# jy-yuan/KIVI

Measured on NVIDIA H100. Metric: decode tokens/sec @ Llama-2-7B bs32 seq4k K2V2, higher is better.
Workload: dtype f16 (fp32 accumulate; 2-bit K / 2-bit V codes)

## Files before the change

include/kivi_b200.h:

```cpp
#ifndef KIVI_B200_H
#define KIVI_B200_H

#include <stdint.h>

#ifdef __cplusplus
extern "C" {
#endif

#define KIVI_OK              0
#define KIVI_ERR_BITS       -1
#define KIVI_ERR_SHAPE      -2
#define KIVI_ERR_GQA        -3
#define KIVI_ERR_GROUP      -4
#define KIVI_ERR_ALIGN      -5
#define KIVI_ERR_NULL       -6
#define KIVI_ERR_LAYOUT     -7
#define KIVI_ERR_CAPACITY   -8
#define KIVI_ERR_UNSUPPORTED -9

#define KIVI_LAYOUT_REFERENCE 0
#define KIVI_LAYOUT_KERNEL    1

int         kivi_version(void);
const char* kivi_error_string(int code);
uint64_t    kivi_launch_count(void);

int kivi_pack_lastdim_f16(const void* x, int64_t rows, int64_t T, int group_size, int bits,
                          void* code, void* scale, void* mn, void* stream);

int kivi_bgemv_outer_f16(const void* A, int64_t a_stride,
                         const void* qB, int64_t qb_unit_stride, int64_t qb_row_stride,
                         const void* scales, const void* zeros, int64_t sz_unit_stride, int64_t sz_row_stride,
                         void* C, int B, int nh, int nh_kv, int K, int N,
                         int bits, int group_size, int layout, void* stream);

int kivi_gemv_inner_f16(const void* in, const void* kernel, const void* scales, const void* zeros,
                        void* out, int Bn, int IC, int OC, int bits, int group_size, int64_t sf_w,
                        void* stream);

int kivi_unpack_dequant_lastdim_f16(const void* code, const void* scale, const void* mn,
                                    int64_t rows, int64_t T, int group_size, int bits,
                                    void* out, void* stream);

#define KIVI_CACHE_OVERLAP_PROLOGUE 1
#define KIVI_CACHE_GQA_CHUNK_SHIFT 4
#define KIVI_CACHE_GQA_CHUNK(g)    ((g) << KIVI_CACHE_GQA_CHUNK_SHIFT)

typedef struct kivi_cache {
    int32_t batch, num_heads, num_kv_heads, head_dim;
    int32_t k_bits, v_bits, group_size, residual_length;
    int32_t k_cap_blocks;
    int32_t v_cap_blocks;
    int32_t v_res_cap;
    int32_t flags;
    void* k_store;
    void* v_store;
    void* k_res;
    void* v_res;
    void* state;
} kivi_cache_t;

int kivi_cache_sizes(int batch, int num_kv_heads, int k_bits, int v_bits, int group_size,
                     int residual_length, int max_tokens, int64_t* out);

int kivi_cache_prefill_f16(const kivi_cache_t* cache, const void* k, const void* v, int n, void* stream);

int64_t kivi_decode_workspace_bytes(const kivi_cache_t* cache, int max_kv_len);

int kivi_decode_attention_f16(const kivi_cache_t* cache, const void* q, const void* k_new, const void* v_new,
                              const void* mask, void* out, void* workspace, int64_t workspace_bytes,
                              void* dbg_logits, void* dbg_probs, int64_t dbg_stride, int max_kv_len, void* stream);

int kivi_decode_attention_ragged_f16(const kivi_cache_t* cache, const void* q, const void* k_new, const void* v_new,
                                     const int32_t* kv_start, const void* mask, void* out, void* workspace,
                                     int64_t workspace_bytes, void* dbg_logits, void* dbg_probs, int64_t dbg_stride,
                                     int max_kv_len, void* stream);

int kivi_debug_range_split(int n_units, int n_b, int n_w, int w_cap, int kernel, int* out_lo, int* out_owner);

int kivi_debug_ragged_items(int n_units, int n_b, int n_w, int w_cap, int kernel, const int* unit_start, int kv_len,
                            int* issued, int* consumed, int64_t cap, int64_t* n_out);

int kivi_cache_advance(const kivi_cache_t* cache, void* stream);

#define KIVI_STATE_ERR_CAPACITY 1
#define KIVI_STATE_ERR_LENGTHS  2
int kivi_cache_read_state(const kivi_cache_t* cache, int32_t* host_state8, void* stream);

int kivi_cache_refill_f16(const kivi_cache_t* cache, int seq, const void* k, const void* v, int n,
                          int tk, int r, int tv, int L, int vhead, void* stream);

int kivi_cache_shift_f16(const kivi_cache_t* cache, int shift, int tk, int tv, void* stream);

int kivi_cache_shift_state(const kivi_cache_t* cache, int shift, int32_t* kv_start, void* stream);

int kivi_cache_export_f16(const kivi_cache_t* cache, int tk, int r, int tv, int L, int vhead,
                          void* k_code, void* k_scale, void* k_mn, void* k_full,
                          void* v_code, void* v_scale, void* v_mn, void* v_full, void* stream);

int kivi_cache_import_f16(const kivi_cache_t* cache, int tk, int r, int tv, int L,
                          const void* k_code, const void* k_scale, const void* k_mn, const void* k_full,
                          const void* v_code, const void* v_scale, const void* v_mn, const void* v_full, void* stream);

int kivi_add_rmsnorm_f16(const void* x, void* residual, const void* weight, void* out,
                         int rows, int hidden, float eps, void* stream);
int kivi_rope_split_f16(const void* qkv, const void* cos_table, const void* sin_table, const void* pos,
                        void* q, void* k, void* v, int batch, int num_heads, int num_kv_heads, int table_rows,
                        void* stream);
int kivi_silu_mul_f16(const void* gate_up, void* out, int rows, int intermediate, void* stream);

int kivi_greedy_sample_exchange_f32(const void* logits, int batch, int vocab, void* next_local, void* ids_feedback,
                                    const void* peer_buffers, int rank, int world, const void* step, void* err, void* stream);

#ifdef __cplusplus
}
#endif
#endif
```

kivi_b200/csrc/kivi_attn.cuh:

```cuda
#pragma once
#include <cstdlib>
#include "kivi_decode.cuh"

#ifndef KIVI_UNROLL
#define KIVI_UNROLL 8
#endif
constexpr int kChunkUnroll = KIVI_UNROLL;
#ifndef KIVI_Z_SIMT
#define KIVI_Z_SIMT 0
#endif
#ifndef KIVI_EVICT_FIRST
#define KIVI_EVICT_FIRST 1
#endif
#ifndef KIVI_SHIFT_IMAD
#define KIVI_SHIFT_IMAD 0
#endif
#ifndef KIVI_PRED_FINALIZE
#define KIVI_PRED_FINALIZE 1
#endif
#ifndef KIVI_EARLY_COMMIT
#define KIVI_EARLY_COMMIT 1
#endif
#ifndef KIVI_UNIT_FLAGS
#define KIVI_UNIT_FLAGS 0
#endif
#ifndef KIVI_COMMIT_IN_QK
#define KIVI_COMMIT_IN_QK 0
#endif
#if KIVI_COMMIT_IN_QK && KIVI_UNIT_FLAGS
#error "KIVI_COMMIT_IN_QK relies on the grid dependency between the two kernels (the ticket reset); KIVI_UNIT_FLAGS removes it"
#endif
#ifndef KIVI_PREFETCH_SV
#define KIVI_PREFETCH_SV 0
#endif
#ifndef KIVI_COMMIT_ASYNC
#define KIVI_COMMIT_ASYNC 0
#endif
#ifndef KIVI_DEFER_ARRIVE
#define KIVI_DEFER_ARRIVE 0
#endif
#ifndef KIVI_Q_FIRST
#define KIVI_Q_FIRST 1
#endif
#ifndef KIVI_REL_ARRIVE
#define KIVI_REL_ARRIVE 0
#endif
#ifndef KIVI_WIN_LOGITS_BULK
#define KIVI_WIN_LOGITS_BULK 1
#endif
#ifndef KIVI_GRID_CONSTANT
#define KIVI_GRID_CONSTANT 1
#endif
#if KIVI_GRID_CONSTANT
#define KIVI_PARAM_QUAL __grid_constant__
#else
#define KIVI_PARAM_QUAL
#endif
template <int G> struct Lat { static constexpr bool q_first = KIVI_Q_FIRST && G == 1, win_bulk = KIVI_WIN_LOGITS_BULK && G == 1; };
#ifndef KIVI_COMMIT_LATE
#define KIVI_COMMIT_LATE 0
#endif

namespace kivi {

int make_desc(const kivi_cache_t* k, CacheDesc* d);

#ifndef KIVI_CW
#define KIVI_CW 16
#endif
constexpr int kCW = KIVI_CW;
#ifndef KIVI_MINB
#define KIVI_MINB (KIVI_CW >= 16 ? 1 : 2)
#endif
#ifndef KIVI_CW_K4G4
#define KIVI_CW_K4G4 12
#endif
template <int KB, int G> struct WarpsPerCta { static constexpr int k = (KB == 4 && G == 4 && KIVI_CW >= 16) ? KIVI_CW_K4G4 : kCW; };
constexpr int kHalfChunks = 8;
constexpr int kParts = 8 / kHalfChunks;
constexpr int kPartTokens = 16 * kHalfChunks;
constexpr int kResTile = 16;
constexpr int kResBytes = kResTile * kD * 2;
constexpr float kRcpSqrtD = 1.0f / 11.313708f;
constexpr float kProbScale = 64.f, kProbScaleInv = 1.f / 64.f;
constexpr float kQPrescaleBelow = 0.125f;

template <int KB>
__device__ __forceinline__ float2 q_prescale(float mx) {
    constexpr int Q = KB == 4 ? 2 : 0;
    if (!(mx > 0.f) || !(mx < kQPrescaleBelow)) return make_float2(1.f, 1.f);
    const int k = Q - ((int)((__float_as_uint(mx) >> 23) & 0xff) - 127);
    return make_float2(__uint_as_float((uint32_t)(127 + k) << 23), __uint_as_float((uint32_t)(127 - k) << 23));
}
__device__ __forceinline__ int pv_boost(float m) {
    if (!(m > 0.f) || !(m < 0.0625f)) return 0;
    return min(-4 - ((int)((__float_as_uint(m) >> 23) & 0xff) - 127), 9);
}
__device__ __forceinline__ int pv_extra_exp(float S, int b) {
    return min(max((int)((__float_as_uint(S) >> 23) & 0xff) - 127, 0), 15) + b;
}
__device__ __forceinline__ __half2 pow2_h2(int e) {
    const uint32_t h = (uint32_t)(15 + e) << 10, hh = h | (h << 16);
    return *reinterpret_cast<const __half2*>(&hh);
}

__device__ __forceinline__ void pdl_wait() { asm volatile("griddepcontrol.wait;" ::: "memory"); }
__device__ __forceinline__ void pdl_trigger() { asm volatile("griddepcontrol.launch_dependents;"); }

#if KIVI_TIMELINE
static __device__ unsigned long long g_timeline[2][4096][8];
__device__ __forceinline__ unsigned long long gtime() { unsigned long long t; asm volatile("mov.u64 %0, %globaltimer;" : "=l"(t)); return t; }
#define KIVI_TL(k, w, i) do { if (lane == 0 && (w) < 4096) { g_timeline[k][w][i] = gtime(); if ((i) == 0) { unsigned sm_; asm volatile("mov.u32 %0, %%smid;" : "=r"(sm_)); g_timeline[k][w][4] = sm_; } } } while (0)
static inline int timeline_fetch(unsigned long long* host_out) {
    return (int)cudaMemcpyFromSymbol(host_out, g_timeline, sizeof(unsigned long long) * 2 * 4096 * 8);
}
#else
#define KIVI_TL(k, w, i) do {} while (0)
#endif

struct Workspace {
    __half* lg; long long ld;
    float2* stats; int stat_cap;
    float* part; int part_cap;
    int* count;
    int* ready;
    int* ticket;
};

struct AttnParams {
    CacheDesc c;
    const __half* q; const __half* k_new; const __half* v_new; const __half* mask;
    const int32_t* kv_start;
    __half* out; __half* dbg_logits; __half* dbg_probs;
    long long dbg_stride;
    Workspace w;
    int stage_bytes, spw , hchunks, n_units, nw_eff ;
    int max_kv_len;
};

struct Sched {
    int tk, r, tv, L, vhead, T, seg1;
    int n_kb, n_kr, n_vb, vr1, n_vr;
    int ipu;
    int bpu;
};

__device__ __forceinline__ Sched make_sched(const CacheDesc& c) {
    Sched s;
    s.tk = c.state[ST_TK]; s.r = c.state[ST_R]; s.tv = c.state[ST_TV]; s.L = c.state[ST_L]; s.vhead = c.state[ST_VHEAD];
    s.T = s.tk + s.r + 1;
    s.n_kb = cdiv(s.tk, kBlockTokens);
    s.n_kr = cdiv(s.r, kResTile);
    s.n_vb = cdiv(s.tv, kBlockTokens);
    s.seg1 = min(s.L, c.v_res_cap - s.vhead);
    s.vr1 = cdiv(s.seg1, kResTile);
    s.n_vr = s.vr1 + cdiv(s.L - s.seg1, kResTile);
    s.ipu = s.n_kb + s.n_kr + 1;
    s.bpu = s.n_vb + s.n_vr + 1;
    return s;
}

__device__ __forceinline__ bool sched_ok(const Sched& s, const CacheDesc& c, int max_kv_len) {
    return s.tk >= 0 && s.tv >= 0 && s.r >= 0 && s.L >= 0 && s.r < c.R && s.L <= c.R && s.T <= max_kv_len &&
           s.tv + 1 <= max_kv_len && s.vhead >= 0 && s.vhead < c.v_res_cap && s.tk % c.R == 0;
}

struct Pipe {
    uint8_t* base; uint64_t* full; int spw, stage_bytes;
    int c_stage, c_par;
    int i_stage;
    __device__ __forceinline__ void init(uint8_t* b, uint64_t* f, int spw_, int sb) {
        base = b; full = f; spw = spw_; stage_bytes = sb; c_stage = 0; c_par = 0; i_stage = 0;
    }
    __device__ __forceinline__ uint8_t* cons() const { return base + (size_t)c_stage * stage_bytes; }
    __device__ __forceinline__ void wait() const { mbar_wait(&full[c_stage], (uint32_t)c_par); }
    __device__ __forceinline__ void pop() { if (++c_stage == spw) { c_stage = 0; c_par ^= 1; } }
    __device__ __forceinline__ uint8_t* prod() const { return base + (size_t)i_stage * stage_bytes; }
    __device__ __forceinline__ uint64_t* prod_bar() const { return &full[i_stage]; }
    __device__ __forceinline__ void push() { if (++i_stage == spw) i_stage = 0; }
};

__device__ __forceinline__ __half scale_logit(float acc) {
    return __float2half_rn(__half2float(__float2half_rn(acc)) * kRcpSqrtD);
}

__device__ __forceinline__ float fast_exp(float x) {
    float y;
    asm("ex2.approx.ftz.f32 %0, %1;" : "=f"(y) : "f"(x * 1.4426950408889634f));
    return y;
}

__device__ __forceinline__ uint32_t h2_as_u32(const __half2 h) { return *reinterpret_cast<const uint32_t*>(&h); }
__device__ __forceinline__ __half2 u32_as_h2(const uint32_t u) { return *reinterpret_cast<const __half2*>(&u); }

#ifndef KIVI_BPREP2
#define KIVI_BPREP2 1
#endif
__device__ __forceinline__ uint32_t b_prep(uint32_t x2, uint32_t s2, __half2 msel) {
    const __half2 x = u32_as_h2(x2), s = u32_as_h2(s2);
#if KIVI_BPREP2
    __half2 b = __hmul2(x, s);
    if (h2_as_u32(msel) != 0u) b = __hfma2(x, s, __hneg2(b));
    return h2_as_u32(b);
#else
    const __half2 nh = __hmul2(__hmul2(x, s), msel);
    return h2_as_u32(__hfma2(x, s, nh));
#endif
}

template <int BITS>
__device__ __forceinline__ float inv_pos_scale(int mm) {
    return __uint_as_float((uint32_t)(127 + 24 - Lay<BITS>::bitpos(mm % Lay<BITS>::F)) << 23);
}

template <int G, int GS>
struct Cols {
    static constexpr int NG = 128 / GS;
    static constexpr int GPF = 4 / G;
    static constexpr int NF = (NG + GPF - 1) / GPF;
};

template <int BITS, int G, int GS, bool INIT, class XF>
__device__ __forceinline__ void mma_half(const uint8_t* st, int c0, XF&& getx, float (&acc)[8][4], float (&zc)[4], int lane)
{
    using L = Lay<BITS>;
    using CL = Cols<G, GS>;
    constexpr int NG = CL::NG, GPF = CL::GPF, NF = CL::NF;
    const int g8 = lane >> 2, t = lane & 3;
    const int hb = (g8 % (2 * G)) >> 1;
    const int gi = g8 / (2 * G);
    const int gz = min(g8 >> 1, NG - 1);
    const __half2 msel = (g8 & 1) ? __float2half2_rn(-1.f) : __float2half2_rn(0.f);
    const uint8_t* meta = st + kHalfChunks * L::kChunkBytes + t * 16;
    constexpr uint32_t kField = ((1u << BITS) - 1u) * 0x00010001u;
    #pragma unroll (kChunkUnroll)
    for (int cl = 0; cl < kHalfChunks; ++cl) {
        uint32_t xa, xb;
        getx(c0 + cl, hb, xa, xb);
        const uint4 mz = *reinterpret_cast<const uint4*>(meta + (cl * NG + gz) * 64);
        if (KIVI_Z_SIMT && G == 1) {
            const float2 x0 = __half22float2(u32_as_h2(xa)), x1 = __half22float2(u32_as_h2(xb));
            const float2 z0 = __half22float2(u32_as_h2(mz.x)), z1 = __half22float2(u32_as_h2(mz.z));
            float zp = (INIT && cl == 0) ? x0.x * z0.x : fmaf(x0.x, z0.x, zc[0]);
            zp = fmaf(x0.y, z0.y, zp); zp = fmaf(x1.x, z1.x, zp); zc[0] = fmaf(x1.y, z1.y, zp);
        } else if (INIT && cl == 0) mma_16816_init(zc, mz.x, mz.y, mz.z, mz.w, xa, xb);
        else mma_16816(zc, mz.x, mz.y, mz.z, mz.w, xa, xb);
        uint32_t b0[NF], b1[NF];
        if (G == 1 && NF == 1) {
            b0[0] = b_prep(xa, mz.y, msel); b1[0] = b_prep(xb, mz.w, msel);
        } else {
            #pragma unroll
            for (int f = 0; f < NF; ++f) {
                const int grp = min(f * GPF + gi, NG - 1);
                const uint4 ms = *reinterpret_cast<const uint4*>(meta + (cl * NG + grp) * 64);
                b0[f] = b_prep(xa, ms.y, msel); b1[f] = b_prep(xb, ms.w, msel);
            }
        }
        #pragma unroll
        for (int sl = 0; sl < L::kSlabs; ++sl) {
            const uint4 w4 = *reinterpret_cast<const uint4*>(st + (cl * L::kSlabs + sl) * 512 + lane * 16);
            const uint32_t w[4] = {w4.x, w4.y, w4.z, w4.w};
            uint32_t wl4[4], wr4[4], wr6[4], wr8[4];
            #pragma unroll
            for (int r = 0; r < 4; ++r) {
#if KIVI_SHIFT_IMAD
                wl4[r] = w[r] << 4; wr4[r] = __umulhi(w[r], 1u << 28); wr6[r] = __umulhi(w[r], 1u << 26); wr8[r] = __umulhi(w[r], 1u << 24);
#else
                wl4[r] = w[r] << 4; wr4[r] = w[r] >> 4; wr6[r] = w[r] >> 6; wr8[r] = w[r] >> 8;
#endif
            }
            #pragma unroll
            for (int j = 0; j < L::F; ++j) {
                uint32_t a[4];
                #pragma unroll
                for (int r = 0; r < 4; ++r) {
                    const int sh = L::shr(j);
                    const uint32_t src = sh == -4 ? wl4[r] : sh == 0 ? w[r] : sh == 4 ? wr4[r] : sh == 6 ? wr6[r] : wr8[r];
                    a[r] = src & (kField << L::bitpos(j));
                }
                const int mm = sl * L::F + j;
                const int f = ((16 * mm) / GS) / GPF;
                if (INIT && cl == 0) mma_16816_init(acc[mm], a[0], a[1], a[2], a[3], b0[f], b1[f]);
                else mma_16816(acc[mm], a[0], a[1], a[2], a[3], b0[f], b1[f]);
            }
        }
    }
}

template <int G, int GS>
__device__ __forceinline__ void gather_z(const float (&zc)[4], int lane, float (&zsel)[Cols<G, GS>::NG]) {
    float z = zc[0];
    if (KIVI_Z_SIMT && G == 1) {
        z += __shfl_xor_sync(0xffffffffu, z, 1);
        z += __shfl_xor_sync(0xffffffffu, z, 2);
    }
#if KIVI_PRED_FINALIZE
    if (G == 1 && GS == 32) {
        const float zt = __shfl_sync(0xffffffffu, z, 9 * (lane & 3));
        #pragma unroll
        for (int grp = 0; grp < Cols<G, GS>::NG; ++grp) zsel[grp] = zt;
        return;
    }
#endif
    #pragma unroll
    for (int grp = 0; grp < Cols<G, GS>::NG; ++grp)
        zsel[grp] = __shfl_sync(0xffffffffu, z, 8 * grp + (lane & 3));
}

__device__ __forceinline__ float selp(float a, float b, bool p) {
    float r;
    asm("{ .reg .pred q; setp.ne.b32 q, %3, 0; selp.f32 %0, %2, %1, q; }" : "=f"(r) : "f"(a), "f"(b), "r"((int)p));
    return r;
}
__device__ __forceinline__ float sel4(float v0, float v1, float v2, float v3, bool t1, bool t2) {
    return selp(selp(v0, v1, t1), selp(v2, v3, t1), t2);
}

template <int G, int GS> struct Slots { static constexpr int k = (G == 1 && GS == 32) ? 4 : 16; };

template <int BITS, int G, int GS, class EF>
__device__ __forceinline__ void finalize(const float (&acc)[8][4], const float (&zsel)[Cols<G, GS>::NG], int lane,
                                         float post, EF&& emit)
{
    constexpr int GPF = Cols<G, GS>::GPF;
    const int g8 = lane >> 2, t = lane & 3;
    if (G == 1 && GS == 32) {
#if KIVI_PRED_FINALIZE
        float v0 = 0.f, v1 = 0.f, v2 = 0.f, v3 = 0.f;
        #pragma unroll
        for (int v = 0; v < 4; ++v) {
            if (t == v) {
                const float sl = inv_pos_scale<BITS>(2 * v) * post, sh = inv_pos_scale<BITS>(2 * v + 1) * post, zt = zsel[v] * post;
                v0 = fmaf(acc[2 * v][0] + acc[2 * v][1], sl, zt);
                v1 = fmaf(acc[2 * v][2] + acc[2 * v][3], sl, zt);
                v2 = fmaf(acc[2 * v + 1][0] + acc[2 * v + 1][1], sh, zt);
                v3 = fmaf(acc[2 * v + 1][2] + acc[2 * v + 1][3], sh, zt);
            }
        }
        const int o = 32 * t + g8;
        emit(0, o, v0);
        emit(1, o + 8, v1);
        emit(2, o + 16, v2);
        emit(3, o + 24, v3);
#else
        const bool t1 = t & 1, t2 = t & 2;
        float lo[4], hi[4];
        #pragma unroll
        for (int e = 0; e < 4; ++e) {
            lo[e] = sel4(acc[0][e], acc[2][e], acc[4][e], acc[6][e], t1, t2);
            hi[e] = sel4(acc[1][e], acc[3][e], acc[5][e], acc[7][e], t1, t2);
        }
        const float sl = sel4(inv_pos_scale<BITS>(0), inv_pos_scale<BITS>(2), inv_pos_scale<BITS>(4), inv_pos_scale<BITS>(6), t1, t2) * post;
        const float sh = sel4(inv_pos_scale<BITS>(1), inv_pos_scale<BITS>(3), inv_pos_scale<BITS>(5), inv_pos_scale<BITS>(7), t1, t2) * post;
        const float zt = sel4(zsel[0], zsel[1], zsel[2], zsel[3], t1, t2) * post;
        const int o = 32 * t + g8;
        emit(0, o, fmaf(lo[0] + lo[1], sl, zt));
        emit(1, o + 8, fmaf(lo[2] + lo[3], sl, zt));
        emit(2, o + 16, fmaf(hi[0] + hi[1], sh, zt));
        emit(3, o + 24, fmaf(hi[2] + hi[3], sh, zt));
#endif
    } else {
        const int gi_l = t / G;
        #pragma unroll
        for (int mm = 0; mm < 8; ++mm) {
            const int grp = (16 * mm) / GS;
            if (grp % GPF == gi_l) {
                const float sc = inv_pos_scale<BITS>(mm) * post, zt = zsel[grp] * post;
                emit(2 * mm, 16 * mm + g8, fmaf(acc[mm][0] + acc[mm][1], sc, zt));
                emit(2 * mm + 1, 16 * mm + g8 + 8, fmaf(acc[mm][2] + acc[mm][3], sc, zt));
            }
        }
    }
}

template <int G, int GS, class EF>
__device__ __forceinline__ void walk_slots(const float (&run)[Slots<G, GS>::k], int lane, EF&& emit)
{
    constexpr int GPF = Cols<G, GS>::GPF;
    const int g8 = lane >> 2, t = lane & 3;
    if (G == 1 && GS == 32) {
        #pragma unroll
        for (int e = 0; e < 4; ++e) emit(32 * t + g8 + 8 * e, run[e]);
    } else {
        const int gi_l = t / G;
        #pragma unroll
        for (int mm = 0; mm < 8; ++mm) {
            if (((16 * mm) / GS) % GPF == gi_l) {
                emit(16 * mm + g8, run[2 * mm]);
                emit(16 * mm + g8 + 8, run[2 * mm + 1]);
            }
        }
    }
}

struct CommitIn { uint4 vnew4, knew4; uint2 vold; };

__device__ __forceinline__ CommitIn commit_fetch(const AttnParams& p, const Sched& s, int u, int lane)
{
    const CacheDesc& c = p.c;
    CommitIn in;
    in.vnew4 = make_uint4(0u, 0u, 0u, 0u); in.knew4 = in.vnew4; in.vold = make_uint2(0u, 0u);
    if (lane < kD / 8) in.vnew4 = __ldg(reinterpret_cast<const uint4*>(p.v_new + (int64_t)u * kD) + lane);
    if (lane >= 16) in.knew4 = __ldg(reinterpret_cast<const uint4*>(p.k_new + (int64_t)u * kD) + (lane - 16));
    if (s.L + 1 > c.R) in.vold = __ldcg(reinterpret_cast<const uint2*>(c.v_res + (int64_t)u * c.v_res_cap * kD + win_off(s.vhead, lane * 4)));
    return in;
}

template <int KB, int VB>
__device__ __noinline__ void commit_unit(const AttnParams& p, const Sched& s, int u, int lane, uint8_t* scratch, const CommitIn& in)
{
    const CacheDesc& c = p.c;
    const int g = c.g;
    const uint4 vnew4 = in.vnew4, knew4 = in.knew4;
    const uint2 vold = in.vold;
    if (lane < kD / 8)
        reinterpret_cast<uint4*>(c.v_res + (int64_t)u * c.v_res_cap * kD)[win_unit((s.vhead + s.L) % c.v_res_cap, lane)] = vnew4;
    if (s.L + 1 > c.R) {
        using VL = Lay<VB>;
        const float maxq = (float)((1 << VB) - 1);
        const int bb = lay_block_bytes(VB, g);
        uint8_t* blk = c.v_store + ((int64_t)u * c.v_cap_blocks + s.tv / kBlockTokens) * bb;
        const int inner = s.tv % kBlockTokens;
        const uint2 raw = vold;
        const __half2* rh = reinterpret_cast<const __half2*>(&raw);
        const float2 x01 = __half22float2(rh[0]), x23 = __half22float2(rh[1]);
        const float x[4] = {x01.x, x01.y, x23.x, x23.y};
        float mnf = fminf(fminf(x[0], x[1]), fminf(x[2], x[3])), mxf = fmaxf(fmaxf(x[0], x[1]), fmaxf(x[2], x[3]));
        const int lpg = g / 4;
        for (int o = 1; o < lpg; o <<= 1) {
            mnf = fminf(mnf, __shfl_xor_sync(0xffffffffu, mnf, o));
            mxf = fmaxf(mxf, __shfl_xor_sync(0xffffffffu, mxf, o));
        }
        const __half sc = quant_scale(mnf, mxf, VB);
        const float scf = __half2float(sc), rcp = __frcp_rn(scf);
        uint32_t four = 0;
        #pragma unroll
        for (int e = 0; e < 4; ++e) four |= quant_code(x[e], mnf, scf, rcp, maxq) << (8 * e);
        __syncwarp();
        reinterpret_cast<uint32_t*>(scratch)[lane] = four;
        if (lane % lpg == 0) {
            *reinterpret_cast<__half*>(blk + lay_scale_off(VB, g, inner, lane / lpg)) = sc;
            *reinterpret_cast<__half*>(blk + lay_zero_off(VB, g, inner, lane / lpg)) = __float2half_rn(mnf);
        }
        __syncwarp();
        if (lane < VL::kSlabs * 16) {
            const int sl = lane >> 4, row = lane & 15;
            uint32_t hw = 0;
            #pragma unroll
            for (int j = 0; j < VL::F; ++j) hw |= (uint32_t)scratch[sl * VL::kSlabRows + 16 * j + row] << (VB * j);
            *reinterpret_cast<uint16_t*>(blk + lay_word_off(VB, inner, sl * VL::kSlabRows + row) + 2 * (inner & 1)) = (uint16_t)hw;
        }
        __syncwarp();
    }
    if (s.r + 1 < c.R) {
        if (lane >= 16) reinterpret_cast<uint4*>(c.k_res + (int64_t)u * c.R * kD)[win_unit(s.r, lane - 16)] = knew4;
    }
}

template <int KB>
__device__ __noinline__ void k_flush_slice(const AttnParams& p, const Sched& s, int u, int q, int lane)
{
    const CacheDesc& c = p.c;
    const int g = c.g;
    const float maxq = (float)((1 << KB) - 1);
    const int bb = lay_block_bytes(KB, g);
    uint8_t* ub = c.k_store + (int64_t)u * c.k_cap_blocks * bb;
    const __half* win = c.k_res + (int64_t)u * c.R * kD;
    const __half* knew = p.k_new + (int64_t)u * kD;
    const int nblk = max(1, c.R / kBlockTokens);
    const int cnt = min(c.R, kBlockTokens);
    const int hw = lane >> 4, cu = lane & 15;
    auto row2 = [&](int t) -> __half2 {
        return t < c.R - 1 ? u32_as_h2(__ldcg(reinterpret_cast<const uint32_t*>(win + (int64_t)t * kD + ((cu ^ (t & 7)) << 3)) + q))
                           : u32_as_h2(__ldg(reinterpret_cast<const uint32_t*>(knew + 8 * cu) + q));
    };
    #pragma unroll 1
    for (int bi = 0; bi < nblk; ++bi) {
        const int tb = s.tk + bi * kBlockTokens;
        const int o0 = tb % kBlockTokens;
        uint8_t* blk = ub + (int64_t)(tb / kBlockTokens) * bb;
        const bool partial = cnt < kBlockTokens;
        uint32_t* wbase = reinterpret_cast<uint32_t*>(blk) + lay_word_inner(KB, 8 * cu + 2 * q);
        uint32_t words[8];
        int cur_sl = -1;
        #pragma unroll 1
        for (int gl = 0; gl < cnt / g; ++gl) {
            const int tl0 = bi * kBlockTokens + gl * g;
            float mn0 = INFINITY, mx0 = -INFINITY, mn1 = INFINITY, mx1 = -INFINITY;
            #pragma unroll 1
            for (int i0 = 0; i0 < g; i0 += 16) {
                __half2 v[8];
                #pragma unroll
                for (int m = 0; m < 8; ++m) v[m] = row2(tl0 + i0 + 2 * m + hw);
                #pragma unroll
                for (int m = 0; m < 8; ++m) {
                    const float2 f = __half22float2(v[m]);
                    mn0 = fminf(mn0, f.x); mx0 = fmaxf(mx0, f.x);
                    mn1 = fminf(mn1, f.y); mx1 = fmaxf(mx1, f.y);
                }
            }
            mn0 = fminf(mn0, __shfl_xor_sync(0xffffffffu, mn0, 16)); mx0 = fmaxf(mx0, __shfl_xor_sync(0xffffffffu, mx0, 16));
            mn1 = fminf(mn1, __shfl_xor_sync(0xffffffffu, mn1, 16)); mx1 = fmaxf(mx1, __shfl_xor_sync(0xffffffffu, mx1, 16));
            const __half sc0 = quant_scale(mn0, mx0, KB), sc1 = quant_scale(mn1, mx1, KB);
            const float scf0 = __half2float(sc0), scf1 = __half2float(sc1), rcp0 = __frcp_rn(scf0), rcp1 = __frcp_rn(scf1);
            const int og = o0 + gl * g;
            if (hw == 0) {
                __align__(8) __half mz[4] = {__float2half_rn(mn0), __float2half_rn(mn1), sc0, sc1};
                *reinterpret_cast<uint2*>(blk + lay_meta_pair_off(KB, g, 8 * cu + 2 * q, og / g)) = *reinterpret_cast<const uint2*>(mz);
            }
            #pragma unroll 1
            for (int q16 = 0; q16 < g / 16; ++q16) {
                const int o = og + 16 * q16;
                const int sl = o / Lay<KB>::kSlabRows, j = (o % Lay<KB>::kSlabRows) / 16;
                if (sl != cur_sl) {
                    if (cur_sl >= 0) {
                        #pragma unroll
                        for (int m = 0; m < 8; ++m) wbase[lay_word_row(cur_sl, 2 * m + hw)] = words[m];
                    }
                    cur_sl = sl;
                    #pragma unroll
                    for (int m = 0; m < 8; ++m) words[m] = partial ? wbase[lay_word_row(sl, 2 * m + hw)] : 0u;
                }
                const uint32_t keep = ~((((1u << KB) - 1u) * 0x00010001u) << (KB * j));
                __half2 v[8];
                #pragma unroll
                for (int m = 0; m < 8; ++m) v[m] = row2(tl0 + 16 * q16 + 2 * m + hw);
                #pragma unroll
                for (int m = 0; m < 8; ++m) {
                    const float2 f = __half22float2(v[m]);
                    const uint32_t c0 = quant_code(f.x, mn0, scf0, rcp0, maxq);
                    const uint32_t c1 = quant_code(f.y, mn1, scf1, rcp1, maxq);
                    words[m] = (words[m] & keep) | ((c0 | (c1 << 16)) << (KB * j));
                }
            }
        }
        if (cur_sl >= 0) {
            #pragma unroll
            for (int m = 0; m < 8; ++m) wbase[lay_word_row(cur_sl, 2 * m + hw)] = words[m];
        }
    }
}

__device__ __forceinline__ void warp_max_sum(float mx, float sm, float& M, float& S) {
    #pragma unroll
    for (int o = 16; o >= 1; o >>= 1) {
        const float mo = __shfl_xor_sync(0xffffffffu, mx, o), so = __shfl_xor_sync(0xffffffffu, sm, o);
        const float mn = fmaxf(mx, mo);
        sm = (mx == -INFINITY ? 0.f : sm * fast_exp(mx - mn)) + (mo == -INFINITY ? 0.f : so * fast_exp(mo - mn));
        mx = mn;
    }
    M = mx; S = sm;
}

__device__ __forceinline__ __half apply_mask(__half v, const __half* mask, int64_t idx) {
    v = __hadd_rn(v, mask[idx]);
    if (__half2float(v) < -65504.f) v = __float2half_rn(-65504.f);
    return v;
}

#ifndef KIVI_UNIFORM_RANGES
#define KIVI_UNIFORM_RANGES 1
#endif
struct CostQK { static constexpr unsigned cb = KIVI_UNIFORM_RANGES ? 1 : 16, cw = KIVI_UNIFORM_RANGES ? 1 : 10,
                                          cn = KIVI_UNIFORM_RANGES ? 1 : 2, cv = KIVI_UNIFORM_RANGES ? 0 : 12; };
struct CostSV { static constexpr unsigned cb = KIVI_UNIFORM_RANGES ? 1 : 16, cw = KIVI_UNIFORM_RANGES ? 1 : 3,
                                          cn = KIVI_UNIFORM_RANGES ? 1 : 12, cv = KIVI_UNIFORM_RANGES ? 0 : 35; };

template <class C>
struct Ranges {
    int n_b, n_w, per_unit;
    unsigned Cu, W; unsigned long long Ctot; int small;
    __host__ __device__ __forceinline__ void init(int n_units, int nb, int nw, long long w_cap) {
        n_b = nb; n_w = nw; per_unit = nb + nw + 1;
        Cu = C::cv + (unsigned)nb * C::cb + (unsigned)nw * C::cw + C::cn;
        Ctot = (unsigned long long)n_units * Cu;
        constexpr unsigned cmax = C::cv + (C::cb > C::cw ? (C::cb > C::cn ? C::cb : C::cn) : (C::cw > C::cn ? C::cw : C::cn));
        const unsigned long long n_items = (unsigned long long)n_units * per_unit;
        unsigned long long w = (unsigned long long)w_cap;
        w = w < Ctot / cmax ? w : Ctot / cmax;
        w = w < n_items ? w : n_items;
        W = (unsigned)(w < 1 ? 1 : w);
        small = (Ctot + Cu) * W < (1ull << 32) ? 1 : 0;
    }
    __host__ __device__ __forceinline__ unsigned kj(int j) const {
        if (j <= 0) return 0u;
        const int jb = min(j, n_b), jw = min(max(j - n_b, 0), n_w);
        return C::cv + (unsigned)jb * C::cb + (unsigned)jw * C::cw + (j > n_b + n_w ? C::cn : 0u);
    }
    __host__ __device__ __forceinline__ int owner(int unit, int j) const {
        if (small) return (int)(((unsigned)unit * Cu + kj(j)) * W / (unsigned)Ctot);
        return (int)(((unsigned long long)unit * Cu + kj(j)) * W / Ctot);
    }
    __host__ __device__ __forceinline__ void lo(int w, int& unit, int& j) const {
        unsigned long long x;
        if (small) x = ((unsigned)w * (unsigned)Ctot + W - 1u) / W;
        else x = ((unsigned long long)w * Ctot + W - 1ull) / W;
        unit = small ? (int)((unsigned)x / Cu) : (int)(x / Cu);
        const unsigned rem = (unsigned)(x - (unsigned long long)unit * Cu);
        if (rem == 0u) { j = 0; return; }
        if (rem <= C::cv) j = 1;
        else {
            const unsigned r = rem - C::cv;
            if (r <= (unsigned)n_b * C::cb) j = (int)((r + C::cb - 1u) / C::cb);
            else if (r <= (unsigned)n_b * C::cb + (unsigned)n_w * C::cw) j = n_b + (int)((r - (unsigned)n_b * C::cb + C::cw - 1u) / C::cw);
            else j = per_unit;
        }
        if (j >= per_unit) { j = 0; ++unit; }
    }
};

struct Cursor {
    int unit, j, half, left;
    int s_unit, s_pos;
};

__host__ __device__ __forceinline__ void cursor_step(Cursor& cur, int per_unit, int n_b) {
    if (cur.j < n_b && cur.half + 1 < kParts) { ++cur.half; return; }
    cur.half = 0;
    --cur.left;
    if (++cur.j == per_unit) { cur.j = 0; ++cur.unit; }
}

__host__ __device__ __forceinline__ int clamp_start(int start, int kv_len) {
    return start < 0 ? 0 : (start > kv_len ? kv_len : start);
}
__host__ __device__ __forceinline__ bool ragged_skip(int j, int n_b, int start) {
    return j < n_b && (j + 1) * kBlockTokens <= start;
}
template <class SF>
__host__ __device__ __forceinline__ bool ragged_seek(Cursor& cur, int per_unit, int n_b, SF&& start_of) {
    while (cur.left > 0) {
        if (cur.j == per_unit - 1) { cur.j = 0; ++cur.unit; --cur.left; }
        else if (cur.half == 0 && ragged_skip(cur.j, n_b, start_of(cur.unit))) { ++cur.j; --cur.left; }
        else return true;
    }
    return false;
}

#ifndef KIVI_EXP_FMA
#define KIVI_EXP_FMA 1
#endif
constexpr float kLog2e = 1.4426950408889634f;
__device__ __forceinline__ float fast_exp_sub(float x, float m, float nml) {
#if KIVI_EXP_FMA
    float y;
    asm("ex2.approx.ftz.f32 %0, %1;" : "=f"(y) : "f"(fmaf(x, kLog2e, nml)));
    (void)m;
    return y;
#else
    (void)nml;
    return fast_exp(x - m);
#endif
}

template <int N_>
__device__ __forceinline__ void fold_stats(float& m, float& s, const float (&x)[N_]) {
    float mn = m;
    #pragma unroll
    for (int e = 0; e < N_; ++e) mn = fmaxf(mn, x[e]);
    if (mn != -INFINITY) {
        float acc = s * fast_exp(m - mn);
        const float nml = -mn * kLog2e;
        #pragma unroll
        for (int e = 0; e < N_; ++e) acc += fast_exp_sub(x[e], mn, nml);
        m = mn; s = acc;
    }
}

__device__ __forceinline__ int unit_start(const AttnParams& p, const Sched& s, int unit) {
    const int u = p.hchunks == 1 ? unit : unit / p.hchunks;
    return clamp_start(__ldg(p.kv_start + u / p.c.Hkv), s.T - 1);
}
__device__ __forceinline__ int cursor_start(Cursor& cur, const AttnParams& p, const Sched& s, int unit) {
    if (unit != cur.s_unit) { cur.s_unit = unit; cur.s_pos = unit_start(p, s, unit); }
    return cur.s_pos;
}

template <int KB, int GS, bool RAGGED>
__device__ __forceinline__ void qk_issue_next(Pipe& pp, Cursor& cur, const AttnParams& p, const Sched& s,
                                              int lane, uint64_t pol)
{
    const CacheDesc& c = p.c;
    if constexpr (RAGGED) {
        if (!ragged_seek(cur, s.ipu, s.n_kb, [&](int un) { return cursor_start(cur, p, s, un); })) return;
    } else {
        if (cur.left > 0 && cur.j == s.ipu - 1) {
            cur.j = 0; ++cur.unit; --cur.left;
        }
        if (cur.left <= 0) return;
    }
    if (lane == 0) {
        const int u = p.hchunks == 1 ? cur.unit : cur.unit / p.hchunks;
        uint8_t* dst = pp.prod();
        uint64_t* bar = pp.prod_bar();
        asm volatile("fence.proxy.async.shared::cta;" ::: "memory");
        if (cur.j < s.n_kb) {
            constexpr int cb = kHalfChunks * Lay<KB>::kChunkBytes;
            const int mb = lay_meta_bytes(GS) / kParts;
            const uint8_t* blk = c.k_store + ((int64_t)u * c.k_cap_blocks + cur.j) * lay_block_bytes(KB, GS);
            mbar_expect_tx(bar, (uint32_t)(cb + mb));
            if (kParts == 1) {
                bulk_g2s(dst, blk, (uint32_t)(cb + mb), bar, pol);
            } else {
                bulk_g2s(dst, blk + cur.half * cb, cb, bar, pol);
                bulk_g2s(dst + cb, blk + kParts * cb + cur.half * mb, (uint32_t)mb, bar, pol);
            }
        } else {
            const int t0 = (cur.j - s.n_kb) * kResTile, nt = min(kResTile, s.r - t0);
            mbar_expect_tx(bar, (uint32_t)(nt * kD * 2));
            bulk_g2s(dst, c.k_res + ((int64_t)u * c.R + t0) * kD, (uint32_t)(nt * kD * 2), bar, pol);
        }
    }
    pp.push();
    cursor_step(cur, s.ipu, s.n_kb);
}

template <int KB, int G, int GS, int CW, bool RAGGED>
__global__ void __launch_bounds__(CW * 32, KIVI_MINB)
qk_kernel(const KIVI_PARAM_QUAL AttnParams p)
{
    constexpr int kCW = CW, kThreads = CW * 32;
    extern __shared__ __align__(128) uint8_t smem[];
    const CacheDesc& c = p.c;
    const int tid = threadIdx.x, warp = tid >> 5, lane = tid & 31;
    const int t4 = lane & 3;
    const int n_stages = kCW * p.spw;
    uint64_t* full_all = reinterpret_cast<uint64_t*>(smem + (size_t)n_stages * p.stage_bytes);
    uint8_t* ptr = smem + (((size_t)n_stages * (p.stage_bytes + 8) + 127) & ~(size_t)127);
    uint2* q2 = reinterpret_cast<uint2*>(ptr) + warp * (G * 32);
    float* qlin = reinterpret_cast<float*>(ptr + kCW * G * 32 * 8) + warp * (G * kD);

    __shared__ Ranges<CostQK> rg_sh;
    const Sched s = make_sched(c);
    if (tid < n_stages) { mbar_init(&full_all[tid], 1); mbar_fence_init(); }
    if (tid == kThreads - 1) rg_sh.init(p.n_units, s.n_kb, s.n_kr, p.nw_eff);
    __syncthreads();
    pdl_trigger();

    const uint64_t pol = KIVI_EVICT_FIRST ? policy_evict_first() : policy_evict_last();
    const int gw = blockIdx.x * kCW + warp;
    if (!sched_ok(s, c, p.max_kv_len)) { if (gw == 0 && lane == 0) c.state[6] = KIVI_STATE_ERR_CAPACITY; return; }
    KIVI_TL(0, gw, 0);
    const Ranges<CostQK>& rg = rg_sh;
    if (gw >= (int)rg.W) { pdl_wait(); return; }
    int u_lo, j_lo, u_hi, j_hi;
    rg.lo(gw, u_lo, j_lo); rg.lo(gw + 1, u_hi, j_hi);
    const int n_mine = (u_hi - u_lo) * s.ipu + (j_hi - j_lo);
    Pipe pp;
    pp.init(smem + (size_t)warp * p.spw * p.stage_bytes, full_all + warp * p.spw, p.spw, p.stage_bytes);
    Cursor cur;
    cur.unit = u_lo; cur.j = j_lo; cur.half = 0; cur.left = n_mine; cur.s_unit = -1; cur.s_pos = 0;
    for (int i = 0; i < (Lat<G>::q_first ? 1 : p.spw); ++i) qk_issue_next<KB, GS, RAGGED>(pp, cur, p, s, lane, pol);

    constexpr int NG = Cols<G, GS>::NG;
    const int ratio = c.H / c.Hkv;
    const int h_l = t4 % G;
    const bool slow = p.mask || p.dbg_logits;

    int unit = u_lo, j = j_lo, left = n_mine;
    uint2 qf[G], ql[G];
    auto fetch_q = [&](int un) {
        const int u_ = p.hchunks == 1 ? un : un / p.hchunks, hc_ = p.hchunks == 1 ? 0 : un % p.hchunks;
        const int row0 = u_ * ratio + hc_ * G;
        #pragma unroll
        for (int h = 0; h < G; ++h) {
            const uint32_t* qh = reinterpret_cast<const uint32_t*>(p.q + (int64_t)(row0 + h) * kD + 16 * (lane >> 2) + 2 * (lane & 3));
            qf[h] = make_uint2(__ldg(qh), __ldg(qh + 4));
            ql[h] = __ldg(reinterpret_cast<const uint2*>(p.q + (int64_t)(row0 + h) * kD) + lane);
        }
    };
    pdl_wait();
    fetch_q(unit);
    if (Lat<G>::q_first)
        for (int i = 1; i < p.spw; ++i) qk_issue_next<KB, GS, RAGGED>(pp, cur, p, s, lane, pol);
    KIVI_TL(0, gw, 1);
    #pragma unroll 1
    while (left > 0) {
        const int u = p.hchunks == 1 ? unit : unit / p.hchunks, hc = p.hchunks == 1 ? 0 : unit % p.hchunks;
        const int b = u / c.Hkv;
        const int uq0 = u * ratio + hc * G;
        const int j_first = j;
        const int n_here = min(left, s.ipu - j);
        const int start = RAGGED ? unit_start(p, s, unit) : 0;

        float qpost_blk = 1.f, qpost_win = 1.f;
        __syncwarp();
        #pragma unroll
        for (int h = 0; h < G; ++h) {
            const __half2* qh = reinterpret_cast<const __half2*>(&ql[h]);
            const float2 a = __half22float2(qh[0]), b2 = __half22float2(qh[1]);
            *reinterpret_cast<float4*>(qlin + h * kD + lane * 4) = make_float4(a.x, a.y, b2.x, b2.y);
            float mx = fmaxf(fmaxf(fabsf(a.x), fabsf(a.y)), fmaxf(fabsf(b2.x), fabsf(b2.y)));
            #pragma unroll
            for (int o = 16; o >= 1; o >>= 1) mx = fmaxf(mx, __shfl_xor_sync(0xffffffffu, mx, o));
            const float2 ps = q_prescale<KB>(mx);
            auto sc = [&](uint32_t w) {
                const float2 f = __half22float2(u32_as_h2(w));
                return h2_as_u32(__floats2half2_rn(f.x * ps.x, f.y * ps.x));
            };
            q2[h * 32 + lane] = make_uint2(sc(qf[h].x), sc(qf[h].y));
            if (h == h_l) qpost_blk = ps.y;
            if (h == (lane >> 2)) qpost_win = ps.y;
        }
        __syncwarp();
        if (left > n_here) fetch_q(unit + 1);

        float m_blk = -INFINITY, s_blk = 0.f, m_win = -INFINITY, s_win = 0.f;

        #pragma unroll 1
        for (int k = 0; k < n_here; ++k, ++j) {
            if constexpr (RAGGED) {
                if (ragged_skip(j, s.n_kb, start)) continue;
            }
            if (j < s.n_kb) {
                float acc[8][4];
                float zc[4];
                if (kParts > 1) {
                    #pragma unroll
                    for (int mm = 0; mm < 8; ++mm)
                        #pragma unroll
                        for (int e = 0; e < 4; ++e) acc[mm][e] = 0.f;
                    #pragma unroll
                    for (int e = 0; e < 4; ++e) zc[e] = 0.f;
                }
                #pragma unroll 1
                for (int half = 0; half < kParts; ++half) {
                    pp.wait();
                    mma_half<KB, G, GS, kParts == 1>(pp.cons(), half * kHalfChunks, [&](int cc, int h, uint32_t& xa, uint32_t& xb) {
                        const uint2 v = q2[(h * 8 + cc) * 4 + t4];
                        xa = v.x; xb = v.y;
                    }, acc, zc, lane);
                    __syncwarp();
                    pp.pop();
                    qk_issue_next<KB, GS, RAGGED>(pp, cur, p, s, lane, pol);
                }
                float zsel[NG];
                gather_z<G, GS>(zc, lane, zsel);
                const int64_t rowi = uq0 + h_l;
                __half* row = p.w.lg + rowi * p.w.ld + j * kBlockTokens;
                const int nvalid = s.tk - j * kBlockTokens;
                const bool padded = RAGGED && j * kBlockTokens < start;
                float x[Slots<G, GS>::k];
                #pragma unroll
                for (int e = 0; e < Slots<G, GS>::k; ++e) x[e] = -INFINITY;
                if (!slow && !padded && nvalid >= kBlockTokens) {
                    finalize<KB, G, GS>(acc, zsel, lane, qpost_blk, [&](int slot, int o, float v) {
                        const __half hv = scale_logit(v);
                        row[o] = hv;
                        x[slot] = __half2float(hv);
                    });
                } else {
                    finalize<KB, G, GS>(acc, zsel, lane, qpost_blk, [&](int slot, int o, float v) {
                        if (o < nvalid) {
                            __half hv = scale_logit(v);
                            if (p.mask) hv = apply_mask(hv, p.mask, (int64_t)b * s.T + j * kBlockTokens + o);
                            row[o] = hv;
                            if (p.dbg_logits) p.dbg_logits[rowi * p.dbg_stride + j * kBlockTokens + o] = hv;
                            if (!padded || j * kBlockTokens + o >= start) x[slot] = __half2float(hv);
                        }
                    });
                }
                fold_stats(m_blk, s_blk, x);
            } else if (j < s.ipu - 1) {
                const int t0 = (j - s.n_kb) * kResTile, nt = min(kResTile, s.r - t0);
                pp.wait();
                const uint8_t* st = pp.cons();
                float d0[4] = {0.f, 0.f, 0.f, 0.f}, d1[4] = {0.f, 0.f, 0.f, 0.f};
                const int g8 = lane >> 2;
                const int key = (t0 + g8) & 7;
                const uint8_t* r0 = st + g8 * 256 + t4 * 4, * r1 = r0 + 8 * 256;
                #pragma unroll
                for (int cc = 0; cc < 8; ++cc) {
                    uint2 qa = make_uint2(0u, 0u);
                    if (g8 < G) qa = q2[(g8 * 8 + cc) * 4 + t4];
                    const int u0 = ((2 * cc) ^ key) * 16, u1 = ((2 * cc + 1) ^ key) * 16;
                    mma_16816(d0, qa.x, 0u, qa.y, 0u, *reinterpret_cast<const uint32_t*>(r0 + u0), *reinterpret_cast<const uint32_t*>(r0 + u1));
                    mma_16816(d1, qa.x, 0u, qa.y, 0u, *reinterpret_cast<const uint32_t*>(r1 + u0), *reinterpret_cast<const uint32_t*>(r1 + u1));
                }
                __syncwarp();
                pp.pop();
                qk_issue_next<KB, GS, RAGGED>(pp, cur, p, s, lane, pol);
                if (g8 < G) {
                    const int64_t rowi = uq0 + g8;
                    float x[4];
                    #pragma unroll
                    for (int e = 0; e < 4; ++e) {
                        const int t = (e >> 1) * 8 + 2 * t4 + (e & 1);
                        x[e] = -INFINITY;
                        if (t < nt) {
                            __half hv = scale_logit((e < 2 ? d0[e] : d1[e - 2]) * qpost_win);
                            if (p.mask) hv = apply_mask(hv, p.mask, (int64_t)b * s.T + s.tk + t0 + t);
                            p.w.lg[rowi * p.w.ld + s.tk + t0 + t] = hv;
                            if (p.dbg_logits) p.dbg_logits[rowi * p.dbg_stride + s.tk + t0 + t] = hv;
                            if (!RAGGED || s.tk + t0 + t >= start) x[e] = __half2float(hv);
                        }
                    }
                    fold_stats(m_win, s_win, x);
                }
            } else {
                const uint2 kv = __ldg(reinterpret_cast<const uint2*>(p.k_new + (int64_t)u * kD) + lane);
                const __half2* kh = reinterpret_cast<const __half2*>(&kv);
                const float2 k01 = __half22float2(kh[0]), k23 = __half22float2(kh[1]);
                #pragma unroll
                for (int h = 0; h < G; ++h) {
                    const float4 qv = *reinterpret_cast<const float4*>(qlin + h * kD + lane * 4);
                    float sum = qv.x * k01.x;
                    sum = fmaf(qv.y, k01.y, sum); sum = fmaf(qv.z, k23.x, sum); sum = fmaf(qv.w, k23.y, sum);
                    sum = warp_sum(sum);
                    if (lane == 4 * h) {
                        __half hv = scale_logit(sum);
                        const int64_t rowi = uq0 + h;
                        if (p.mask) hv = apply_mask(hv, p.mask, (int64_t)b * s.T + s.T - 1);
                        p.w.lg[rowi * p.w.ld + s.T - 1] = hv;
                        if (p.dbg_logits) p.dbg_logits[rowi * p.dbg_stride + s.T - 1] = hv;
                        const float x1[1] = {__half2float(hv)};
                        fold_stats(m_win, s_win, x1);
                    }
                }
            }
        }

        const int w_first = rg.owner(unit, 0);
        #pragma unroll
        for (int h = 0; h < G; ++h) {
            float m = -INFINITY, sm = 0.f;
            if ((lane >> 2) == h) { m = m_win; sm = s_win; }
            if (h_l == h && m_blk != -INFINITY) {
                const float mn = fmaxf(m, m_blk);
                sm = (m == -INFINITY ? 0.f : sm * fast_exp(m - mn)) + s_blk * fast_exp(m_blk - mn);
                m = mn;
            }
            float M, S;
            warp_max_sum(m, sm, M, S);
            if (lane == 0) p.w.stats[(int64_t)(uq0 + h) * p.w.stat_cap + (gw - w_first)] = make_float2(M, S);
        }
#if KIVI_UNIT_FLAGS
        __syncwarp();
        if (lane == 0) asm volatile("red.release.gpu.global.add.s32 [%0], 1;" ::"l"(p.w.ready + unit) : "memory");
#endif
        (void)j_first;
        left -= n_here;
        if (j == s.ipu) { j = 0; ++unit; }
    }
    KIVI_TL(0, gw, 2);
#if KIVI_COMMIT_IN_QK && KIVI_EARLY_COMMIT
    {
        const int nu = c.B * c.Hkv;
        uint8_t* scratch = reinterpret_cast<uint8_t*>(qlin);
        #pragma unroll 1
        for (;;) {
            int t = 0;
            if (lane == 0) t = atomicAdd(p.w.ticket, 1);
            t = __shfl_sync(0xffffffffu, t, 0);
            if (t >= nu) break;
            if (c.v_bits == 2) commit_unit<KB, 2>(p, s, t, lane, scratch, commit_fetch(p, s, t, lane));
            else commit_unit<KB, 4>(p, s, t, lane, scratch, commit_fetch(p, s, t, lane));
        }
    }
#endif
#if KIVI_PREFETCH_SV
    {
        Ranges<CostSV> rs;
        rs.init(p.n_units, s.n_vb, s.n_vr, p.nw_eff);
        if (gw < (int)rs.W) {
            int pu, pj;
            rs.lo(gw, pu, pj);
            #pragma unroll 1
            for (int i = 0; i < KIVI_PREFETCH_SV && pu < p.n_units; ++i) {
                if (pj < s.n_vb) {
                    if (lane == 0) {
                        const int u_ = p.hchunks == 1 ? pu : pu / p.hchunks;
                        bulk_prefetch_l2(c.v_store + ((int64_t)u_ * c.v_cap_blocks + pj) * lay_block_bytes(c.v_bits, GS),
                                         (uint32_t)lay_block_bytes(c.v_bits, GS));
                    }
                    ++pj;
                } else { pj = 0; ++pu; }
            }
        }
    }
#endif
    KIVI_TL(0, gw, 3);
}

__device__ __forceinline__ void wait_unit_ready(const AttnParams& p, const Sched& s, const Ranges<CostQK>& rq, int un, int lane)
{
#if KIVI_UNIT_FLAGS
    if (lane == 0) {
        const int need = rq.owner(un, s.ipu - 1) - rq.owner(un, 0) + 1;
        int have;
        do {
            asm volatile("ld.acquire.gpu.global.s32 %0, [%1];" : "=r"(have) : "l"(p.w.ready + un) : "memory");
            if (have < need) __nanosleep(40);
        } while (have < need);
        asm volatile("fence.proxy.async;" ::: "memory");
    }
    __syncwarp();
#endif
}

template <int VB, int G, int GS, bool RAGGED>
__device__ __forceinline__ void sv_issue_next(Pipe& pp, Cursor& cur, const AttnParams& p, const Sched& s,
                                              int ratio, int lane, uint64_t pol, const Ranges<CostQK>& rq, int& ready_unit)
{
    const CacheDesc& c = p.c;
    if constexpr (RAGGED) {
        if (!ragged_seek(cur, s.bpu, s.n_vb, [&](int un) { return cursor_start(cur, p, s, un); })) return;
    } else {
        if (cur.left > 0 && cur.j == s.bpu - 1) {
            cur.j = 0; ++cur.unit; --cur.left;
        }
        if (cur.left <= 0) return;
    }
    if (cur.unit != ready_unit) { wait_unit_ready(p, s, rq, cur.unit, lane); ready_unit = cur.unit; }
    if (lane == 0) {
        const int u = p.hchunks == 1 ? cur.unit : cur.unit / p.hchunks, hc = p.hchunks == 1 ? 0 : cur.unit % p.hchunks;
        uint8_t* dst = pp.prod();
        uint64_t* bar = pp.prod_bar();
        asm volatile("fence.proxy.async.shared::cta;" ::: "memory");
        if (cur.j < s.n_vb) {
            constexpr int cb = kHalfChunks * Lay<VB>::kChunkBytes;
            const int mb = lay_meta_bytes(GS) / kParts;
            const uint8_t* blk = c.v_store + ((int64_t)u * c.v_cap_blocks + cur.j) * lay_block_bytes(VB, GS);
            mbar_expect_tx(bar, (uint32_t)(cb + mb + G * kPartTokens * 2));
            if (kParts == 1) {
                bulk_g2s(dst, blk, (uint32_t)(cb + mb), bar, pol);
            } else {
                bulk_g2s(dst, blk + cur.half * cb, cb, bar, pol);
                bulk_g2s(dst + cb, blk + kParts * cb + cur.half * mb, (uint32_t)mb, bar, pol);
            }
            const int uq0 = u * ratio + hc * G;
            for (int h = 0; h < G; ++h)
                bulk_g2s(dst + cb + mb + h * kPartTokens * 2,
                         p.w.lg + (int64_t)(uq0 + h) * p.w.ld + cur.j * kBlockTokens + cur.half * kPartTokens,
                         kPartTokens * 2, bar, pol);
        } else {
            const int i = cur.j - s.n_vb;
            int slot0, nt;
            if (i < s.vr1) { const int t0 = i * kResTile; slot0 = s.vhead + t0; nt = min(kResTile, s.seg1 - t0); }
            else { const int t0 = (i - s.vr1) * kResTile; slot0 = t0; nt = min(kResTile, s.L - s.seg1 - t0); }
            if (Lat<G>::win_bulk && p.spw >= 2) {
                mbar_expect_tx(bar, (uint32_t)(nt * kD * 2 + G * 48));
                bulk_g2s(dst, c.v_res + ((int64_t)u * c.v_res_cap + slot0) * kD, (uint32_t)(nt * kD * 2), bar, pol);
                const int l0 = i < s.vr1 ? i * kResTile : s.seg1 + (i - s.vr1) * kResTile;
                const int uq0 = u * ratio + hc * G;
                for (int h = 0; h < G; ++h) {
                    const int64_t e0 = ((int64_t)(uq0 + h) * p.w.ld + s.tv + l0) & ~(int64_t)7;
                    bulk_g2s(dst + kResBytes + h * 64, p.w.lg + e0, 48u, bar, pol);
                }
            } else {
                mbar_expect_tx(bar, (uint32_t)(nt * kD * 2));
                bulk_g2s(dst, c.v_res + ((int64_t)u * c.v_res_cap + slot0) * kD, (uint32_t)(nt * kD * 2), bar, pol);
            }
        }
    }
    pp.push();
    cursor_step(cur, s.bpu, s.n_vb);
}

__device__ __forceinline__ float prob_f32(float x, float M, float nMl, float S, float rS) {
    const float e = fast_exp_sub(x, M, nMl);
    const float q = e * rS;
    return fmaf(fmaf(-q, S, e), rS, q);
}

template <int KB, int VB, int G, int GS, int CW, bool RAGGED>
__global__ void __launch_bounds__(CW * 32, KIVI_MINB)
sv_kernel(const KIVI_PARAM_QUAL AttnParams p)
{
    constexpr int kCW = CW, kThreads = CW * 32;
    extern __shared__ __align__(128) uint8_t smem[];
    const CacheDesc& c = p.c;
    const int tid = threadIdx.x, warp = tid >> 5, lane = tid & 31;
    const int t4 = lane & 3;
    const int n_stages = kCW * p.spw;
    uint64_t* full_all = reinterpret_cast<uint64_t*>(smem + (size_t)n_stages * p.stage_bytes);
    uint8_t* ptr = smem + (((size_t)n_stages * (p.stage_bytes + 8) + 127) & ~(size_t)127);
    float* obuf = reinterpret_cast<float*>(ptr) + warp * (G * kD);
    uint8_t* scratch = reinterpret_cast<uint8_t*>(obuf);
    (void)scratch;

    __shared__ Ranges<CostSV> rg_sh;
    __shared__ Ranges<CostQK> rq_sh;
    const Sched s = make_sched(c);
    if (tid < n_stages) { mbar_init(&full_all[tid], 1); mbar_fence_init(); }
    if (tid == kThreads - 1) rg_sh.init(p.n_units, s.n_vb, s.n_vr, p.nw_eff);
    if (tid == kThreads - 33) rq_sh.init(p.n_units, s.n_kb, s.n_kr, p.nw_eff);
    __syncthreads();

    const uint64_t pol = KIVI_EVICT_FIRST ? policy_evict_first() : policy_evict_last();
    const int gw = blockIdx.x * kCW + warp;
    if (!sched_ok(s, c, p.max_kv_len)) return;
    KIVI_TL(1, gw, 0);
    const Ranges<CostSV>& rg = rg_sh;
    const Ranges<CostQK>& rq = rq_sh;
    if (gw >= (int)rg.W) return;
    int u_lo, j_lo, u_hi, j_hi;
    rg.lo(gw, u_lo, j_lo); rg.lo(gw + 1, u_hi, j_hi);
    const int n_mine = (u_hi - u_lo) * s.bpu + (j_hi - j_lo);
    const int ratio = c.H / c.Hkv;
    Pipe pp;
    pp.init(smem + (size_t)warp * p.spw * p.stage_bytes, full_all + warp * p.spw, p.spw, p.stage_bytes);
    Cursor cur;
    cur.unit = u_lo; cur.j = j_lo; cur.half = 0; cur.left = n_mine; cur.s_unit = -1; cur.s_pos = 0;
    int ready_unit = -1;
    if (s.r + 1 == c.R) {
        const int n_slices = 4 * c.B * c.Hkv, n_workers = (int)rg.W;
        for (int sl = gw; sl < n_slices; sl += n_workers) k_flush_slice<KB>(p, s, sl >> 2, sl & 3, lane);
    }
#if !KIVI_COMMIT_IN_QK
    auto commit_share = [&]() {
        const long long nu = (long long)c.B * c.Hkv, nwk = (long long)rg.W;
        const int u0 = (int)((gw * nu + nwk - 1) / nwk), u1 = (int)(((gw + 1) * nu + nwk - 1) / nwk);
        for (int uu = u0; uu < u1; ++uu) commit_unit<KB, VB>(p, s, uu, lane, scratch, commit_fetch(p, s, uu, lane));
    };
#endif
#if KIVI_EARLY_COMMIT && !KIVI_COMMIT_LATE && !KIVI_COMMIT_IN_QK
#if KIVI_COMMIT_ASYNC
    if (p.spw < 2) commit_share();
#else
    commit_share();
#endif
#endif
#if !KIVI_UNIT_FLAGS
    pdl_wait();
#endif
#if KIVI_COMMIT_IN_QK && KIVI_EARLY_COMMIT
    if (gw == 0 && lane == 0) *p.w.ticket = 0;
#endif

    constexpr int NG = Cols<G, GS>::NG;
    const int h_l = t4 % G;
    constexpr int kHalfBytes = kHalfChunks * Lay<VB>::kChunkBytes + kHalfChunks * NG * 64;
    const int rec = G * 2 * kD;

    int unit = u_lo, j = j_lo, left = n_mine;
    float2 sn[G];
    int nstat = 0;
    auto fetch_stats = [&](int un) {
        const int u_ = p.hchunks == 1 ? un : un / p.hchunks, hc_ = p.hchunks == 1 ? 0 : un % p.hchunks;
        const int row0 = u_ * ratio + hc_ * G;
        nstat = rq.owner(un, s.ipu - 1) - rq.owner(un, 0) + 1;
        if (un != ready_unit) { wait_unit_ready(p, s, rq, un, lane); ready_unit = un; }
        #pragma unroll
        for (int h = 0; h < G; ++h) {
            sn[h] = make_float2(-INFINITY, 0.f);
            if (lane < nstat) sn[h] = __ldcg(p.w.stats + (int64_t)(row0 + h) * p.w.stat_cap + lane);
        }
    };
    fetch_stats(unit);
#if KIVI_COMMIT_ASYNC && KIVI_EARLY_COMMIT && !KIVI_COMMIT_LATE && !KIVI_COMMIT_IN_QK
    const long long cnu = (long long)c.B * c.Hkv, cnw = (long long)rg.W;
    const int cu0 = (int)((gw * cnu + cnw - 1) / cnw), cu1 = (int)(((gw + 1) * cnu + cnw - 1) / cnw);
    const bool commit_async = p.spw >= 2 && cu1 > cu0;
    if (commit_async) {
        if (lane == 0) {
            uint8_t* dst = pp.prod();
            uint64_t* bar = pp.prod_bar();
            const bool vq = s.L + 1 > c.R;
            mbar_expect_tx(bar, vq ? 768u : 512u);
            bulk_g2s_plain(dst, p.v_new + (int64_t)cu0 * kD, 256u, bar);
            bulk_g2s_plain(dst + 256, p.k_new + (int64_t)cu0 * kD, 256u, bar);
            if (vq) bulk_g2s_plain(dst + 512, c.v_res + ((int64_t)cu0 * c.v_res_cap + s.vhead) * kD, 256u, bar);
        }
        pp.push();
    }
    for (int i = commit_async ? 1 : 0; i < p.spw; ++i) sv_issue_next<VB, G, GS, RAGGED>(pp, cur, p, s, ratio, lane, pol, rq, ready_unit);
    KIVI_TL(1, gw, 1);
    if (commit_async) {
        pp.wait();
        const uint8_t* st = pp.cons();
        CommitIn in;
        in.vnew4 = make_uint4(0u, 0u, 0u, 0u); in.knew4 = in.vnew4; in.vold = make_uint2(0u, 0u);
        if (lane < kD / 8) in.vnew4 = reinterpret_cast<const uint4*>(st)[lane];
        if (lane >= 16) in.knew4 = reinterpret_cast<const uint4*>(st + 256)[lane - 16];
        if (s.L + 1 > c.R) in.vold = *reinterpret_cast<const uint2*>(st + 512 + 2 * (win_off(s.vhead, lane * 4) - s.vhead * kD));
        __syncwarp();
        pp.pop();
        sv_issue_next<VB, G, GS, RAGGED>(pp, cur, p, s, ratio, lane, pol, rq, ready_unit);
        commit_unit<KB, VB>(p, s, cu0, lane, scratch, in);
        for (int uu = cu0 + 1; uu < cu1; ++uu) commit_unit<KB, VB>(p, s, uu, lane, scratch, commit_fetch(p, s, uu, lane));
    }
#else
    for (int i = 0; i < p.spw; ++i) sv_issue_next<VB, G, GS, RAGGED>(pp, cur, p, s, ratio, lane, pol, rq, ready_unit);
    KIVI_TL(1, gw, 1);
#if KIVI_EARLY_COMMIT && KIVI_COMMIT_LATE && !KIVI_COMMIT_IN_QK
    commit_share();
#endif
#endif
    int pend_unit = -1, pend_old = 0, pend_nparts = 0;
    constexpr bool kDefer = KIVI_DEFER_ARRIVE && G == 1;
    int arr_unit = -1, arr_nparts = 0;
    auto do_arrive = [&](int un, int np) {
        __syncwarp();
        if (lane == 0) {
#if KIVI_REL_ARRIVE
            asm volatile("atom.add.release.gpu.global.s32 %0, [%1], 1;" : "=r"(pend_old) : "l"(p.w.count + un) : "memory");
#else
            asm volatile("atom.add.acq_rel.gpu.global.s32 %0, [%1], 1;" : "=r"(pend_old) : "l"(p.w.count + un) : "memory");
#endif
        }
        pend_unit = un; pend_nparts = np;
    };
    CommitIn pend_cin = {};
    auto finish_unit = [&](int un, int nparts, const CommitIn& cin) {
        const int u = p.hchunks == 1 ? un : un / p.hchunks, hc = p.hchunks == 1 ? 0 : un % p.hchunks;
        const int uq0 = u * ratio + hc * G;
#if KIVI_REL_ARRIVE
        if (nparts > 1 && lane == 0) asm volatile("fence.acq_rel.gpu;" ::: "memory");
#endif
        __syncwarp();
        if (nparts > 1 && lane == 0) p.w.count[un] = 0;
#if KIVI_UNIT_FLAGS
        if (lane == 0) p.w.ready[un] = 0;
#endif
        float qs[G][4], rs[G][4];
        #pragma unroll
        for (int h = 0; h < G; ++h)
            #pragma unroll
            for (int e = 0; e < 4; ++e) { qs[h][e] = 0.f; rs[h][e] = 0.f; }
        const float* r0 = p.w.part + (int64_t)un * p.w.part_cap * rec;
        constexpr int kBatch = G == 1 ? 4 : 2;
        #pragma unroll 1
        for (int w0 = 0; w0 < nparts; w0 += kBatch) {
            float4 a[kBatch][G], b4[kBatch][G];
            #pragma unroll
            for (int k = 0; k < kBatch; ++k)
                #pragma unroll
                for (int h = 0; h < G; ++h) {
                    a[k][h] = make_float4(0.f, 0.f, 0.f, 0.f); b4[k][h] = a[k][h];
                    if (w0 + k < nparts) {
                        a[k][h] = __ldcg(reinterpret_cast<const float4*>(r0 + (int64_t)(w0 + k) * rec + (h * 2 + 0) * kD) + lane);
                        b4[k][h] = __ldcg(reinterpret_cast<const float4*>(r0 + (int64_t)(w0 + k) * rec + (h * 2 + 1) * kD) + lane);
                    }
                }
            #pragma unroll
            for (int k = 0; k < kBatch; ++k)
                #pragma unroll
                for (int h = 0; h < G; ++h) {
                    qs[h][0] += a[k][h].x; qs[h][1] += a[k][h].y; qs[h][2] += a[k][h].z; qs[h][3] += a[k][h].w;
                    rs[h][0] += b4[k][h].x; rs[h][1] += b4[k][h].y; rs[h][2] += b4[k][h].z; rs[h][3] += b4[k][h].w;
                }
        }
        #pragma unroll
        for (int h = 0; h < G; ++h) {
            __align__(8) __half o4[4];
            #pragma unroll
            for (int e = 0; e < 4; ++e) {
                __half o = __float2half_rn(rs[h][e]);
                if (s.tv > 0) o = __hadd_rn(__float2half_rn(qs[h][e]), o);
                o4[e] = o;
            }
            *reinterpret_cast<uint2*>(p.out + (int64_t)(uq0 + h) * kD + lane * 4) = *reinterpret_cast<const uint2*>(o4);
        }
#if !KIVI_EARLY_COMMIT
        if (hc == 0) commit_unit<KB, VB>(p, s, u, lane, scratch, cin);
#else
        (void)u; (void)cin;
#endif
    };
    #pragma unroll 1
    while (left > 0) {
        const int u = p.hchunks == 1 ? unit : unit / p.hchunks, hc = p.hchunks == 1 ? 0 : unit % p.hchunks;
        const int uq0 = u * ratio + hc * G;
        const int n_here = min(left, s.bpu - j);
        const int start = RAGGED ? unit_start(p, s, unit) : 0;

        float M[G], S[G], rS[G], nMl[G];
        #pragma unroll
        for (int h = 0; h < G; ++h) {
            float mx = sn[h].x, sm = sn[h].y;
            const float2* st = p.w.stats + (int64_t)(uq0 + h) * p.w.stat_cap;
            for (int i = lane + 32; i < nstat; i += 32) {
                const float2 v = __ldcg(st + i);
                const float mn = fmaxf(mx, v.x);
                sm = (mx == -INFINITY ? 0.f : sm * fast_exp(mx - mn)) + (v.x == -INFINITY ? 0.f : v.y * fast_exp(v.x - mn));
                mx = mn;
            }
            warp_max_sum(mx, sm, M[h], S[h]);
            nMl[h] = -M[h] * kLog2e;
            rS[h] = __frcp_rn(S[h]);
        }
        if (left > n_here) fetch_stats(unit + 1);

        float run[Slots<G, GS>::k];
        float orr[G][4];
        #pragma unroll
        for (int e = 0; e < Slots<G, GS>::k; ++e) run[e] = 0.f;
        #pragma unroll
        for (int h = 0; h < G; ++h)
            #pragma unroll
            for (int e = 0; e < 4; ++e) orr[h][e] = 0.f;

        #pragma unroll 1
        for (int k = 0; k < n_here; ++k, ++j) {
            if constexpr (RAGGED) {
                if (ragged_skip(j, s.n_vb, start)) continue;
            }
            if (j < s.n_vb) {
                float acc[8][4];
                float zc[4];
                if (kParts > 1) {
                    #pragma unroll
                    for (int mm = 0; mm < 8; ++mm)
                        #pragma unroll
                        for (int e = 0; e < 4; ++e) acc[mm][e] = 0.f;
                    #pragma unroll
                    for (int e = 0; e < 4; ++e) zc[e] = 0.f;
                }
                static_assert(kParts == 1, "the probability scale of a block (pv_boost) is chosen from the whole block's scales");
                int boost = 0;
                #pragma unroll 1
                for (int half = 0; half < kParts; ++half) {
                    const int t0 = j * kBlockTokens + half * kPartTokens, nt = s.tv - t0;
                    pp.wait();
                    uint8_t* st = pp.cons();
                    __half* prob = reinterpret_cast<__half*>(st + kHalfBytes);
                    {
                        const uint4* mt = reinterpret_cast<const uint4*>(st + kHalfChunks * Lay<VB>::kChunkBytes);
                        const __half h0 = __float2half_rn(0.f);
                        __half2 m2 = __half2half2(h0);
                        #pragma unroll
                        for (int i = 0; i < NG; ++i) {
                            const int idx = lane + 32 * i;
                            const uint4 w = mt[idx];
                            __half2 sa = __habs2(u32_as_h2(w.y)), sb = __habs2(u32_as_h2(w.w));
                            if (nt < kPartTokens) {
                                const int tok = 16 * ((idx >> 2) / NG) + 2 * (idx & 3);
                                sa = __halves2half2(tok < nt ? __low2half(sa) : h0, tok + 1 < nt ? __high2half(sa) : h0);
                                sb = __halves2half2(tok + 8 < nt ? __low2half(sb) : h0, tok + 9 < nt ? __high2half(sb) : h0);
                            }
                            m2 = __hmax2(m2, __hmax2(sa, sb));
                        }
                        float m = fmaxf(__low2float(m2), __high2float(m2));
                        #pragma unroll
                        for (int o = 16; o >= 1; o >>= 1) m = fmaxf(m, __shfl_xor_sync(0xffffffffu, m, o));
                        boost = pv_boost(m);
                        if (lane == 0) *reinterpret_cast<volatile int*>(obuf) = boost;
                    }
                    #pragma unroll
                    for (int h = 0; h < G; ++h) {
                        const int E = 6 + (boost ? pv_extra_exp(S[h], boost) : 0), E1 = min(E, 15);
                        const __half2 f1 = pow2_h2(E1), f2 = pow2_h2(E - E1);
                        #pragma unroll
                        for (int e = 0; e < kPartTokens / 64; ++e) {
                            const int tt = (e * 32 + lane) * 2;
                            const float2 f = __half22float2(*reinterpret_cast<const __half2*>(prob + h * kPartTokens + tt));
                            __half2 pr = __floats2half2_rn(prob_f32(f.x, M[h], nMl[h], S[h], rS[h]), prob_f32(f.y, M[h], nMl[h], S[h], rS[h]));
                            if (tt >= nt) pr = __float2half2_rn(0.f);
                            else if (tt + 1 >= nt) pr = __halves2half2(__low2half(pr), __float2half_rn(0.f));
                            if constexpr (RAGGED) {
                                if (t0 + tt + 1 < start) pr = __float2half2_rn(0.f);
                                else if (t0 + tt < start) pr = __halves2half2(__float2half_rn(0.f), __high2half(pr));
                            }
                            if (p.dbg_probs) {
                                if (tt < nt) p.dbg_probs[(int64_t)(uq0 + h) * p.dbg_stride + t0 + tt] = __low2half(pr);
                                if (tt + 1 < nt) p.dbg_probs[(int64_t)(uq0 + h) * p.dbg_stride + t0 + tt + 1] = __high2half(pr);
                            }
                            pr = __hmul2(pr, f1);
                            if (boost) pr = __hmul2(pr, f2);
                            *reinterpret_cast<__half2*>(prob + h * kPartTokens + tt) = pr;
                        }
                    }
                    __syncwarp();
                    mma_half<VB, G, GS, kParts == 1>(st, half * kHalfChunks, [&](int cc, int h, uint32_t& xa, uint32_t& xb) {
                        const __half* pr = prob + h * kPartTokens + 16 * (cc - half * kHalfChunks) + 2 * t4;
                        xa = *reinterpret_cast<const uint32_t*>(pr);
                        xb = *reinterpret_cast<const uint32_t*>(pr + 8);
                    }, acc, zc, lane);
                    __syncwarp();
                    pp.pop();
                    sv_issue_next<VB, G, GS, RAGGED>(pp, cur, p, s, ratio, lane, pol, rq, ready_unit);
                }
                float zsel[NG];
                gather_z<G, GS>(zc, lane, zsel);
                const int boost_b = *reinterpret_cast<volatile const int*>(obuf);
                __syncwarp();
                if (!boost_b) {
                    finalize<VB, G, GS>(acc, zsel, lane, 1.f, [&](int slot, int, float v) { run[slot] += v; });
                } else {
                    float post = 0.f;
                    #pragma unroll
                    for (int h = 0; h < G; ++h)
                        if (h == h_l) post = __uint_as_float((uint32_t)(127 - pv_extra_exp(S[h], boost_b)) << 23);
                    finalize<VB, G, GS>(acc, zsel, lane, post, [&](int slot, int, float v) { run[slot] += v; });
                }
            } else if (j < s.bpu - 1) {
                const int i = j - s.n_vb;
                int l0, nt, slot0;
                if (i < s.vr1) { l0 = i * kResTile; nt = min(kResTile, s.seg1 - l0); slot0 = s.vhead + l0; }
                else { const int tt0 = (i - s.vr1) * kResTile; l0 = s.seg1 + tt0; nt = min(kResTile, s.L - s.seg1 - tt0); slot0 = tt0; }
                const bool win_bulk = Lat<G>::win_bulk && p.spw >= 2;
                if (win_bulk) pp.wait();
                uint8_t* st = pp.cons();
                float pl[G];
                #pragma unroll
                for (int h = 0; h < G; ++h) {
                    pl[h] = 0.f;
                    if (lane < nt) {
                        float x;
                        if (win_bulk) {
                            const int off = (int)(((int64_t)(uq0 + h) * p.w.ld + s.tv + l0) & 7);
                            x = __half2float(reinterpret_cast<const __half*>(st + kResBytes + h * 64)[off + lane]);
                        } else {
                            x = __half2float(__ldcg(p.w.lg + (int64_t)(uq0 + h) * p.w.ld + s.tv + l0 + lane));
                        }
                        __half pr = __float2half_rn(prob_f32(x, M[h], nMl[h], S[h], rS[h]));
                        if (RAGGED && s.tv + l0 + lane < start) pr = __float2half_rn(0.f);
                        if (p.dbg_probs) p.dbg_probs[(int64_t)(uq0 + h) * p.dbg_stride + s.tv + l0 + lane] = pr;
                        pl[h] = __half2float(pr);
                    }
                }
                const int g8 = lane >> 2;
                uint32_t b0 = 0u, b1 = 0u;
                #pragma unroll
                for (int h = 0; h < G; ++h) {
                    const float p0 = __shfl_sync(0xffffffffu, pl[h], 2 * t4), p1 = __shfl_sync(0xffffffffu, pl[h], 2 * t4 + 1);
                    const float p2 = __shfl_sync(0xffffffffu, pl[h], 2 * t4 + 8), p3 = __shfl_sync(0xffffffffu, pl[h], 2 * t4 + 9);
                    if (g8 == h) { b0 = h2_as_u32(__floats2half2_rn(p0, p1)); b1 = h2_as_u32(__floats2half2_rn(p2, p3)); }
                }
                if (!win_bulk) pp.wait();
                if (nt < kResTile) {
                    for (int idx = lane; idx < (kResTile - nt) * 16; idx += 32)
                        *reinterpret_cast<uint4*>(st + nt * 256 + idx * 16) = make_uint4(0u, 0u, 0u, 0u);
                    __syncwarp();
                }
                const int tr = ((lane >> 4) << 3) + (lane & 7);
                const uint8_t* rowp = st + tr * 256;
                const int key = (slot0 + tr) & 7, usel = (lane >> 3) & 1;
                float oacc[8][4];
                #pragma unroll
                for (int mt = 0; mt < 8; ++mt) {
                    #pragma unroll
                    for (int e = 0; e < 4; ++e) oacc[mt][e] = 0.f;
                    uint32_t af[4];
                    ldmatrix_x4_trans(af, rowp + (((2 * mt + usel) ^ key) << 4));
                    mma_16816(oacc[mt], af[0], af[1], af[2], af[3], b0, b1);
                }
                __syncwarp();
                pp.pop();
                sv_issue_next<VB, G, GS, RAGGED>(pp, cur, p, s, ratio, lane, pol, rq, ready_unit);
                #pragma unroll
                for (int mt = 0; mt < 8; ++mt)
                    #pragma unroll
                    for (int e = 0; e < 2; ++e)
                        if (2 * t4 + e < G) {
                            obuf[(2 * t4 + e) * kD + 16 * mt + g8] = oacc[mt][e];
                            obuf[(2 * t4 + e) * kD + 16 * mt + g8 + 8] = oacc[mt][2 + e];
                        }
                __syncwarp();
                #pragma unroll
                for (int h = 0; h < G; ++h) {
                    const float4 v = *reinterpret_cast<const float4*>(obuf + h * kD + lane * 4);
                    orr[h][0] += v.x; orr[h][1] += v.y; orr[h][2] += v.z; orr[h][3] += v.w;
                }
                __syncwarp();
            } else {
                const uint2 vv = __ldg(reinterpret_cast<const uint2*>(p.v_new + (int64_t)u * kD) + lane);
                const __half2* vh = reinterpret_cast<const __half2*>(&vv);
                const float2 v01 = __half22float2(vh[0]), v23 = __half22float2(vh[1]);
                #pragma unroll
                for (int h = 0; h < G; ++h) {
                    const float x = __half2float(__ldcg(p.w.lg + (int64_t)(uq0 + h) * p.w.ld + s.T - 1));
                    const __half prh = __float2half_rn(prob_f32(x, M[h], nMl[h], S[h], rS[h]));
                    if (p.dbg_probs && lane == 0) p.dbg_probs[(int64_t)(uq0 + h) * p.dbg_stride + s.T - 1] = prh;
                    const float pr = __half2float(prh);
                    orr[h][0] = fmaf(pr, v01.x, orr[h][0]); orr[h][1] = fmaf(pr, v01.y, orr[h][1]);
                    orr[h][2] = fmaf(pr, v23.x, orr[h][2]); orr[h][3] = fmaf(pr, v23.y, orr[h][3]);
                }
            }
            if (kDefer && arr_unit >= 0) { do_arrive(arr_unit, arr_nparts); arr_unit = -1; }
        }

        const int w_first = rg.owner(unit, 0), w_last = rg.owner(unit, s.bpu - 1);
        const int nparts = w_last - w_first + 1;
        float* recp = p.w.part + ((int64_t)unit * p.w.part_cap + (gw - w_first)) * rec;
        {
            float* rq = recp + (h_l * 2 + 0) * kD;
            walk_slots<G, GS>(run, lane, [&](int o, float v) { rq[o] = v * kProbScaleInv; });
            #pragma unroll
            for (int h = 0; h < G; ++h)
                *reinterpret_cast<float4*>(recp + (h * 2 + 1) * kD + lane * 4) = make_float4(orr[h][0], orr[h][1], orr[h][2], orr[h][3]);
        }
        if (pend_unit >= 0 && __shfl_sync(0xffffffffu, pend_old, 0) == pend_nparts - 1) finish_unit(pend_unit, pend_nparts, pend_cin);
        pend_unit = -1;
#if !KIVI_EARLY_COMMIT
        pend_cin = commit_fetch(p, s, u, lane);
#endif
        if (nparts > 1) {
            if (kDefer && left > n_here) { arr_unit = unit; arr_nparts = nparts; }
            else do_arrive(unit, nparts);
        } else {
            __syncwarp();
            finish_unit(unit, 1, pend_cin);
        }
        left -= n_here;
        if (j == s.bpu) { j = 0; ++unit; }
    }
    KIVI_TL(1, gw, 2);
    if (pend_unit >= 0 && __shfl_sync(0xffffffffu, pend_old, 0) == pend_nparts - 1) finish_unit(pend_unit, pend_nparts, pend_cin);
    KIVI_TL(1, gw, 3);
}

constexpr int kMaxCtasPerSm = KIVI_MINB;

static inline int64_t carve_workspace(const CacheDesc& c, int n_units, int G, int max_kv_len, void* base, Workspace* w)
{
    DeviceInfo di;
    const int drc = device_info(&di);
    if (drc) return drc < 0 ? drc : -(int64_t)drc;
    const int64_t rows = (int64_t)c.B * c.H;
    const int64_t ld = ((int64_t)max_kv_len + 16 + 127) / 128 * 128 + 128;
    const int bpu_max = cdiv(max_kv_len, kBlockTokens) + cdiv(c.R + 1, kResTile) + 4;
    const int warps = di.num_sms * kMaxCtasPerSm * kCW;
    const int part_cap = min(bpu_max, cdiv(warps, n_units) + 2);
    int64_t off = 0;
    auto take = [&](int64_t bytes) { const int64_t o = off; off += (bytes + 255) / 256 * 256; return o; };
    const int64_t o_lg = take(rows * ld * 2);
    const int stat_cap = part_cap;
    const int64_t o_st = take(rows * stat_cap * 8);
    const int64_t o_pt = take((int64_t)n_units * part_cap * G * 2 * kD * 4);
    const int64_t o_ct = take((int64_t)n_units * 4);
    const int64_t o_rd = take((int64_t)n_units * 4);
    const int64_t o_tk = take(4);
    if (w) {
        uint8_t* b = (uint8_t*)base;
        w->lg = (__half*)(b + o_lg); w->ld = ld;
        w->stats = (float2*)(b + o_st); w->stat_cap = stat_cap;
        w->part = (float*)(b + o_pt); w->part_cap = part_cap;
        w->count = (int*)(b + o_ct);
        w->ready = (int*)(b + o_rd);
        w->ticket = (int*)(b + o_tk);
    }
    return off;
}

template <int KB, int VB, int G, int GS, bool RAGGED>
static int launch_attention(AttnParams& p, bool overlap_prologue, cudaStream_t st)
{
    const CacheDesc& c = p.c;
    DeviceInfo di;
    int rc = device_info(&di);
    if (rc) return rc;
    const Tuning& tn = tuning();
    constexpr int kCW = WarpsPerCta<KB, G>::k, kThreads = kCW * 32;
    const int max_smem = di.max_smem_optin - 1024;
    const int half_k = kHalfChunks * Lay<KB>::kChunkBytes + lay_meta_bytes(c.g) / kParts;
    const int half_v = kHalfChunks * Lay<VB>::kChunkBytes + lay_meta_bytes(c.g) / kParts + G * kPartTokens * 2;
    const int stage = max(max(half_k, half_v), kResBytes + G * 64);
    p.stage_bytes = (stage + 127) / 128 * 128;
    const int fixed = 512 + kCW * G * (32 * 8 + kD * 4);
    int ctas = kMaxCtasPerSm;
    p.spw = 0;
    for (; ctas >= 1; --ctas) {
        p.spw = min(4, (max_smem / ctas - fixed) / (kCW * p.stage_bytes));
        if (p.spw >= 2) break;
    }
    if (ctas < 1) { ctas = 1; p.spw = (max_smem - fixed) / (kCW * p.stage_bytes); }
    if (tn.ctas_per_sm >= 1 && tn.ctas_per_sm <= ctas) {
        ctas = tn.ctas_per_sm;
        p.spw = min(8, (max_smem / ctas - fixed) / (kCW * p.stage_bytes));
    }
    if (tn.stages_per_warp >= 1 && tn.stages_per_warp <= p.spw) p.spw = tn.stages_per_warp;
    if (p.spw < 1) return KIVI_ERR_CAPACITY;
    const size_t smem = (size_t)kCW * p.spw * p.stage_bytes + fixed;
    auto kqk = qk_kernel<KB, G, GS, kCW, RAGGED>;
    auto ksv = sv_kernel<KB, VB, G, GS, kCW, RAGGED>;
    static std::atomic<unsigned long long> optin_qk{0}, optin_sv{0};
    rc = ensure_dynamic_smem(kqk, max_smem, di.ordinal, optin_qk); if (rc) return rc;
    rc = ensure_dynamic_smem(ksv, max_smem, di.ordinal, optin_sv); if (rc) return rc;
    const int grid = di.num_sms * ctas;
    const long long want = (long long)p.n_units * max(1, p.w.part_cap - 2);
    p.nw_eff = (int)min((long long)grid * kCW, want);
    const bool pdl = !tn.no_pdl;
    cudaLaunchAttribute attr_qk[1], attr_sv[1];
    attr_qk[0].id = attr_sv[0].id = cudaLaunchAttributeProgrammaticStreamSerialization;
    attr_qk[0].val.programmaticStreamSerializationAllowed = pdl && overlap_prologue ? 1 : 0;
    attr_sv[0].val.programmaticStreamSerializationAllowed = pdl ? 1 : 0;
    cudaLaunchConfig_t cfg = {};
    cfg.gridDim = dim3(grid); cfg.blockDim = dim3(kThreads); cfg.dynamicSmemBytes = smem; cfg.stream = st;
    cfg.attrs = attr_qk; cfg.numAttrs = 1;
    cudaError_t e = cudaLaunchKernelEx(&cfg, kqk, p);
    if (e != cudaSuccess) return (int)e;
    rc = post_launch(); if (rc) return rc;
    cfg.attrs = attr_sv;
    e = cudaLaunchKernelEx(&cfg, ksv, p);
    if (e != cudaSuccess) return (int)e;
    return post_launch();
}

template <int KB, int VB, bool RAGGED>
static int dispatch_attention_g(AttnParams& p, int G, bool overlap_prologue, cudaStream_t st)
{
    #define KIVI_GS(GS_)                                                                  \
        if (p.c.g == GS_) {                                                               \
            if (G == 4) return launch_attention<KB, VB, 4, GS_, RAGGED>(p, overlap_prologue, st);           \
            if (G == 2) return launch_attention<KB, VB, 2, GS_, RAGGED>(p, overlap_prologue, st);           \
            return launch_attention<KB, VB, 1, GS_, RAGGED>(p, overlap_prologue, st);                       \
        }
    KIVI_GS(32)
    KIVI_GS(64)
    KIVI_GS(128)
    #undef KIVI_GS
    return KIVI_ERR_GROUP;
}

template <int KB, int VB>
static int dispatch_attention(AttnParams& p, int G, bool overlap_prologue, cudaStream_t st)
{
    if (p.kv_start) return dispatch_attention_g<KB, VB, true>(p, G, overlap_prologue, st);
    return dispatch_attention_g<KB, VB, false>(p, G, overlap_prologue, st);
}

}
```

kivi_b200/csrc/kivi_decode.cu:

```cuda
#include <cstdlib>
#include "kivi_attn.cuh"

namespace kivi {
int attention_k2v2(AttnParams& p, int G, bool overlap_prologue, cudaStream_t st);
int attention_k4v4(AttnParams& p, int G, bool overlap_prologue, cudaStream_t st);
int attention_k2v4(AttnParams& p, int G, bool overlap_prologue, cudaStream_t st);
int attention_k4v2(AttnParams& p, int G, bool overlap_prologue, cudaStream_t st);
}

using namespace kivi;

static int gqa_chunk(int ratio, int flags) {
    int G = ratio % 4 == 0 ? 4 : (ratio % 2 == 0 ? 2 : 1);
    const int want = (flags >> KIVI_CACHE_GQA_CHUNK_SHIFT) & 7;
    if ((want == 1 || want == 2 || want == 4) && ratio % want == 0) G = want;
    return G;
}

extern "C" int64_t kivi_decode_workspace_bytes(const kivi_cache_t* cache, int max_kv_len)
{
    CacheDesc c;
    int rc = make_desc(cache, &c);
    if (rc) return rc;
    if (max_kv_len <= 0) return KIVI_ERR_SHAPE;
    const int ratio = c.H / c.Hkv, G = gqa_chunk(ratio, cache->flags);
    return carve_workspace(c, c.B * c.Hkv * (ratio / G), G, max_kv_len, nullptr, nullptr);
}

static int decode_attention(const kivi_cache_t* cache, const void* q, const void* k_new, const void* v_new,
                            const int32_t* kv_start, const void* mask, void* out, void* workspace, int64_t workspace_bytes,
                            void* dbg_logits, void* dbg_probs, int64_t dbg_stride, int max_kv_len, void* stream)
{
    AttnParams p;
    int rc = make_desc(cache, &p.c);
    if (rc) return rc;
    if (!q || !k_new || !v_new || !out || !workspace) return KIVI_ERR_NULL;
    if (max_kv_len <= 0) return KIVI_ERR_SHAPE;
    if (max_kv_len > p.c.k_cap_blocks * kBlockTokens) return KIVI_ERR_CAPACITY;
    if (reinterpret_cast<uintptr_t>(workspace) % 256 != 0) return KIVI_ERR_ALIGN;
    if (reinterpret_cast<uintptr_t>(kv_start) % 4 != 0) return KIVI_ERR_ALIGN;
    p.q = (const __half*)q; p.k_new = (const __half*)k_new; p.v_new = (const __half*)v_new; p.mask = (const __half*)mask;
    p.kv_start = kv_start;
    p.out = (__half*)out; p.dbg_logits = (__half*)dbg_logits; p.dbg_probs = (__half*)dbg_probs; p.dbg_stride = dbg_stride;
    const bool overlap = (cache->flags & KIVI_CACHE_OVERLAP_PROLOGUE) != 0;
    const int ratio = p.c.H / p.c.Hkv;
    const int G = gqa_chunk(ratio, cache->flags);
    p.hchunks = ratio / G;
    p.n_units = p.c.B * p.c.Hkv * p.hchunks;
    p.max_kv_len = max_kv_len;
    const int64_t need = carve_workspace(p.c, p.n_units, G, max_kv_len, workspace, &p.w);
    if (need < 0) return (int)need;
    if (need > workspace_bytes) return KIVI_ERR_CAPACITY;
    cudaStream_t st = (cudaStream_t)stream;
    if (p.c.k_bits == 2 && p.c.v_bits == 2) return attention_k2v2(p, G, overlap, st);
    if (p.c.k_bits == 4 && p.c.v_bits == 4) return attention_k4v4(p, G, overlap, st);
    if (p.c.k_bits == 2 && p.c.v_bits == 4) return attention_k2v4(p, G, overlap, st);
    if (p.c.k_bits == 4 && p.c.v_bits == 2) return attention_k4v2(p, G, overlap, st);
    return KIVI_ERR_BITS;
}

extern "C" int kivi_decode_attention_f16(const kivi_cache_t* cache, const void* q, const void* k_new, const void* v_new,
                                         const void* mask, void* out, void* workspace, int64_t workspace_bytes,
                                         void* dbg_logits, void* dbg_probs, int64_t dbg_stride, int max_kv_len, void* stream)
{
    return decode_attention(cache, q, k_new, v_new, nullptr, mask, out, workspace, workspace_bytes, dbg_logits, dbg_probs,
                            dbg_stride, max_kv_len, stream);
}

extern "C" int kivi_decode_attention_ragged_f16(const kivi_cache_t* cache, const void* q, const void* k_new, const void* v_new,
                                                const int32_t* kv_start, const void* mask, void* out, void* workspace,
                                                int64_t workspace_bytes, void* dbg_logits, void* dbg_probs, int64_t dbg_stride,
                                                int max_kv_len, void* stream)
{
    return decode_attention(cache, q, k_new, v_new, kv_start, mask, out, workspace, workspace_bytes, dbg_logits, dbg_probs,
                            dbg_stride, max_kv_len, stream);
}

extern "C" int kivi_debug_range_split(int n_units, int n_b, int n_w, int w_cap, int kernel, int* out_lo, int* out_owner)
{
    if (n_units <= 0 || n_b < 0 || n_w < 0 || w_cap <= 0 || !out_lo) return KIVI_ERR_SHAPE;
    auto run = [&](auto rg) {
        for (int w = 0; w <= (int)rg.W; ++w) rg.lo(w, out_lo[2 * w], out_lo[2 * w + 1]);
        if (out_owner)
            for (int u = 0; u < n_units; ++u)
                for (int j = 0; j < rg.per_unit; ++j) out_owner[(long long)u * rg.per_unit + j] = rg.owner(u, j);
        return (int)rg.W;
    };
    if (kernel == 0) { Ranges<CostQK> rg; rg.init(n_units, n_b, n_w, w_cap); return run(rg); }
    Ranges<CostSV> rg; rg.init(n_units, n_b, n_w, w_cap);
    return run(rg);
}

extern "C" int kivi_debug_ragged_items(int n_units, int n_b, int n_w, int w_cap, int kernel, const int* unit_start, int kv_len,
                                       int* issued, int* consumed, int64_t cap, int64_t* n_out)
{
    if (n_units <= 0 || n_b < 0 || n_w < 0 || w_cap <= 0 || kv_len < 0) return KIVI_ERR_SHAPE;
    if (!unit_start || !issued || !consumed || !n_out) return KIVI_ERR_NULL;
    auto run = [&](auto rg) -> int {
        const int per_unit = rg.per_unit;
        auto start_of = [&](int un) { return clamp_start(unit_start[un], kv_len); };
        int64_t ni = 0, nc = 0;
        auto put = [&](int* dst, int64_t& n, int w, int u, int j, int h) {
            if (n >= cap) return false;
            dst[4 * n] = w; dst[4 * n + 1] = u; dst[4 * n + 2] = j; dst[4 * n + 3] = h;
            ++n;
            return true;
        };
        for (int w = 0; w < (int)rg.W; ++w) {
            int u_lo, j_lo, u_hi, j_hi;
            rg.lo(w, u_lo, j_lo); rg.lo(w + 1, u_hi, j_hi);
            const int n_mine = (u_hi - u_lo) * per_unit + (j_hi - j_lo);
            Cursor cur;
            cur.unit = u_lo; cur.j = j_lo; cur.half = 0; cur.left = n_mine; cur.s_unit = -1; cur.s_pos = 0;
            while (ragged_seek(cur, per_unit, n_b, start_of)) {
                if (!put(issued, ni, w, cur.unit, cur.j, cur.half)) return KIVI_ERR_CAPACITY;
                cursor_step(cur, per_unit, n_b);
            }
            int unit = u_lo, j = j_lo, left = n_mine;
            while (left > 0) {
                const int n_here = left < per_unit - j ? left : per_unit - j;
                const int start = start_of(unit);
                for (int k = 0; k < n_here; ++k, ++j) {
                    if (ragged_skip(j, n_b, start)) continue;
                    if (j < n_b) {
                        for (int h = 0; h < kParts; ++h)
                            if (!put(consumed, nc, w, unit, j, h)) return KIVI_ERR_CAPACITY;
                    } else if (j < per_unit - 1) {
                        if (!put(consumed, nc, w, unit, j, 0)) return KIVI_ERR_CAPACITY;
                    }
                }
                left -= n_here;
                if (j == per_unit) { j = 0; ++unit; }
            }
        }
        n_out[0] = ni; n_out[1] = nc;
        return (int)rg.W;
    };
    if (kernel == 0) { Ranges<CostQK> rg; rg.init(n_units, n_b, n_w, w_cap); return run(rg); }
    Ranges<CostSV> rg; rg.init(n_units, n_b, n_w, w_cap);
    return run(rg);
}

#if KIVI_TIMELINE
#include <vector>
namespace kivi {
int timeline_k2v2(unsigned long long*); int timeline_k2v4(unsigned long long*);
int timeline_k4v2(unsigned long long*); int timeline_k4v4(unsigned long long*);
}
extern "C" int kivi_debug_timeline(unsigned long long* host_out)
{
    const size_t n = 2 * 4096 * 8;
    std::vector<unsigned long long> tmp(n);
    for (size_t i = 0; i < n; ++i) host_out[i] = 0;
    int (*fetch[4])(unsigned long long*) = {timeline_k2v2, timeline_k2v4, timeline_k4v2, timeline_k4v4};
    for (auto f : fetch) {
        const int rc = f(tmp.data());
        if (rc) return rc;
        for (size_t i = 0; i < n; ++i) if (tmp[i] > host_out[i]) host_out[i] = tmp[i];
    }
    return 0;
}
#endif
```

Before: 2830.

## Add fused single-launch per-unit attention kernel for non-ragged MHA decode

Adds a unit_kernel where each warp owns a whole (batch, kv-head) unit. Within one launch it runs the QK pass, folds the softmax max/sum statistics in registers, then runs the SV pass and writes the output directly. A host heuristic selects this path when G==1, the batch is non-ragged and the unit count nearly fills num_sms*8 warps. This removes the second kernel launch, the global stats round-trip and the cross-kernel readiness waits. QK and SV are refactored into reusable range helpers, and the K flush is widened to handle several slices per call. The trade-off is that each unit runs serially on one warp, so load balance depends on units matching warp count, and shared memory per CTA grows with the extra obuf and acc buffers.

```diff
diff --git a/include/kivi_b200.h b/include/kivi_b200.h
--- a/include/kivi_b200.h
+++ b/include/kivi_b200.h
@@ -81,6 +81,9 @@
 int kivi_debug_ragged_items(int n_units, int n_b, int n_w, int w_cap, int kernel, const int* unit_start, int kv_len,
                             int* issued, int* consumed, int64_t cap, int64_t* n_out);
 
+int kivi_debug_attention_path(int n_units, int num_sms, int G, int ragged);
+int kivi_debug_force_attention_path(int mode);
+
 int kivi_cache_advance(const kivi_cache_t* cache, void* stream);
 
 #define KIVI_STATE_ERR_CAPACITY 1
diff --git a/kivi_b200/csrc/kivi_attn.cuh b/kivi_b200/csrc/kivi_attn.cuh
--- a/kivi_b200/csrc/kivi_attn.cuh
+++ b/kivi_b200/csrc/kivi_attn.cuh
@@ -457,8 +457,8 @@
     }
 }
 
-template <int KB>
-__device__ __noinline__ void k_flush_slice(const AttnParams& p, const Sched& s, int u, int q, int lane)
+template <int KB, int NQ>
+__device__ __noinline__ void k_flush_slices(const AttnParams& p, const Sched& s, int u, int q0, int lane)
 {
     const CacheDesc& c = p.c;
     const int g = c.g;
@@ -470,7 +470,7 @@
     const int nblk = max(1, c.R / kBlockTokens);
     const int cnt = min(c.R, kBlockTokens);
     const int hw = lane >> 4, cu = lane & 15;
-    auto row2 = [&](int t) -> __half2 {
+    auto row2 = [&](int t, int q) -> __half2 {
         return t < c.R - 1 ? u32_as_h2(__ldcg(reinterpret_cast<const uint32_t*>(win + (int64_t)t * kD + ((cu ^ (t & 7)) << 3)) + q))
                            : u32_as_h2(__ldg(reinterpret_cast<const uint32_t*>(knew + 8 * cu) + q));
     };
@@ -480,33 +480,46 @@
         const int o0 = tb % kBlockTokens;
         uint8_t* blk = ub + (int64_t)(tb / kBlockTokens) * bb;
         const bool partial = cnt < kBlockTokens;
-        uint32_t* wbase = reinterpret_cast<uint32_t*>(blk) + lay_word_inner(KB, 8 * cu + 2 * q);
-        uint32_t words[8];
+        uint32_t* wbase[NQ];
+        #pragma unroll
+        for (int i = 0; i < NQ; ++i) wbase[i] = reinterpret_cast<uint32_t*>(blk) + lay_word_inner(KB, 8 * cu + 2 * (q0 + i));
+        uint32_t words[NQ][8];
         int cur_sl = -1;
         #pragma unroll 1
         for (int gl = 0; gl < cnt / g; ++gl) {
             const int tl0 = bi * kBlockTokens + gl * g;
-            float mn0 = INFINITY, mx0 = -INFINITY, mn1 = INFINITY, mx1 = -INFINITY;
+            float mn0[NQ], mx0[NQ], mn1[NQ], mx1[NQ];
+            #pragma unroll
+            for (int i = 0; i < NQ; ++i) { mn0[i] = INFINITY; mx0[i] = -INFINITY; mn1[i] = INFINITY; mx1[i] = -INFINITY; }
             #pragma unroll 1
             for (int i0 = 0; i0 < g; i0 += 16) {
-                __half2 v[8];
+                __half2 v[NQ][8];
                 #pragma unroll
-                for (int m = 0; m < 8; ++m) v[m] = row2(tl0 + i0 + 2 * m + hw);
+                for (int m = 0; m < 8; ++m)
+                    #pragma unroll
+                    for (int i = 0; i < NQ; ++i) v[i][m] = row2(tl0 + i0 + 2 * m + hw, q0 + i);
                 #pragma unroll
-                for (int m = 0; m < 8; ++m) {
-                    const float2 f = __half22float2(v[m]);
-                    mn0 = fminf(mn0, f.x); mx0 = fmaxf(mx0, f.x);
-                    mn1 = fminf(mn1, f.y); mx1 = fmaxf(mx1, f.y);
-                }
-            }
-            mn0 = fminf(mn0, __shfl_xor_sync(0xffffffffu, mn0, 16)); mx0 = fmaxf(mx0, __shfl_xor_sync(0xffffffffu, mx0, 16));
-            mn1 = fminf(mn1, __shfl_xor_sync(0xffffffffu, mn1, 16)); mx1 = fmaxf(mx1, __shfl_xor_sync(0xffffffffu, mx1, 16));
-            const __half sc0 = quant_scale(mn0, mx0, KB), sc1 = quant_scale(mn1, mx1, KB);
-            const float scf0 = __half2float(sc0), scf1 = __half2float(sc1), rcp0 = __frcp_rn(scf0), rcp1 = __frcp_rn(scf1);
+                for (int i = 0; i < NQ; ++i)
+                    #pragma unroll
+                    for (int m = 0; m < 8; ++m) {
+                        const float2 f = __half22float2(v[i][m]);
+                        mn0[i] = fminf(mn0[i], f.x); mx0[i] = fmaxf(mx0[i], f.x);
+                        mn1[i] = fminf(mn1[i], f.y); mx1[i] = fmaxf(mx1[i], f.y);
+                    }
+            }
+            __half sc0[NQ], sc1[NQ];
+            float scf0[NQ], scf1[NQ], rcp0[NQ], rcp1[NQ];
             const int og = o0 + gl * g;
-            if (hw == 0) {
-                __align__(8) __half mz[4] = {__float2half_rn(mn0), __float2half_rn(mn1), sc0, sc1};
-                *reinterpret_cast<uint2*>(blk + lay_meta_pair_off(KB, g, 8 * cu + 2 * q, og / g)) = *reinterpret_cast<const uint2*>(mz);
+            #pragma unroll
+            for (int i = 0; i < NQ; ++i) {
+                mn0[i] = fminf(mn0[i], __shfl_xor_sync(0xffffffffu, mn0[i], 16)); mx0[i] = fmaxf(mx0[i], __shfl_xor_sync(0xffffffffu, mx0[i], 16));
+                mn1[i] = fminf(mn1[i], __shfl_xor_sync(0xffffffffu, mn1[i], 16)); mx1[i] = fmaxf(mx1[i], __shfl_xor_sync(0xffffffffu, mx1[i], 16));
+                sc0[i] = quant_scale(mn0[i], mx0[i], KB); sc1[i] = quant_scale(mn1[i], mx1[i], KB);
+                scf0[i] = __half2float(sc0[i]); scf1[i] = __half2float(sc1[i]); rcp0[i] = __frcp_rn(scf0[i]); rcp1[i] = __frcp_rn(scf1[i]);
+                if (hw == 0) {
+                    __align__(8) __half mz[4] = {__float2half_rn(mn0[i]), __float2half_rn(mn1[i]), sc0[i], sc1[i]};
+                    *reinterpret_cast<uint2*>(blk + lay_meta_pair_off(KB, g, 8 * cu + 2 * (q0 + i), og / g)) = *reinterpret_cast<const uint2*>(mz);
+                }
             }
             #pragma unroll 1
             for (int q16 = 0; q16 < g / 16; ++q16) {
@@ -515,28 +528,38 @@
                 if (sl != cur_sl) {
                     if (cur_sl >= 0) {
                         #pragma unroll
-                        for (int m = 0; m < 8; ++m) wbase[lay_word_row(cur_sl, 2 * m + hw)] = words[m];
+                        for (int i = 0; i < NQ; ++i)
+                            #pragma unroll
+                            for (int m = 0; m < 8; ++m) wbase[i][lay_word_row(cur_sl, 2 * m + hw)] = words[i][m];
                     }
                     cur_sl = sl;
                     #pragma unroll
-                    for (int m = 0; m < 8; ++m) words[m] = partial ? wbase[lay_word_row(sl, 2 * m + hw)] : 0u;
+                    for (int i = 0; i < NQ; ++i)
+                        #pragma unroll
+                        for (int m = 0; m < 8; ++m) words[i][m] = partial ? wbase[i][lay_word_row(sl, 2 * m + hw)] : 0u;
                 }
                 const uint32_t keep = ~((((1u << KB) - 1u) * 0x00010001u) << (KB * j));
-                __half2 v[8];
+                __half2 v[NQ][8];
                 #pragma unroll
-                for (int m = 0; m < 8; ++m) v[m] = row2(tl0 + 16 * q16 + 2 * m + hw);
+                for (int m = 0; m < 8; ++m)
+                    #pragma unroll
+                    for (int i = 0; i < NQ; ++i) v[i][m] = row2(tl0 + 16 * q16 + 2 * m + hw, q0 + i);
                 #pragma unroll
-                for (int m = 0; m < 8; ++m) {
-                    const float2 f = __half22float2(v[m]);
-                    const uint32_t c0 = quant_code(f.x, mn0, scf0, rcp0, maxq);
-                    const uint32_t c1 = quant_code(f.y, mn1, scf1, rcp1, maxq);
-                    words[m] = (words[m] & keep) | ((c0 | (c1 << 16)) << (KB * j));
-                }
+                for (int i = 0; i < NQ; ++i)
+                    #pragma unroll
+                    for (int m = 0; m < 8; ++m) {
+                        const float2 f = __half22float2(v[i][m]);
+                        const uint32_t c0 = quant_code(f.x, mn0[i], scf0[i], rcp0[i], maxq);
+                        const uint32_t c1 = quant_code(f.y, mn1[i], scf1[i], rcp1[i], maxq);
+                        words[i][m] = (words[i][m] & keep) | ((c0 | (c1 << 16)) << (KB * j));
+                    }
             }
         }
         if (cur_sl >= 0) {
             #pragma unroll
-            for (int m = 0; m < 8; ++m) wbase[lay_word_row(cur_sl, 2 * m + hw)] = words[m];
+            for (int i = 0; i < NQ; ++i)
+                #pragma unroll
+                for (int m = 0; m < 8; ++m) wbase[i][lay_word_row(cur_sl, 2 * m + hw)] = words[i][m];
         }
     }
 }
@@ -715,49 +738,17 @@
     cursor_step(cur, s.ipu, s.n_kb);
 }
 
-template <int KB, int G, int GS, int CW, bool RAGGED>
-__global__ void __launch_bounds__(CW * 32, KIVI_MINB)
-qk_kernel(const KIVI_PARAM_QUAL AttnParams p)
-{
-    constexpr int kCW = CW, kThreads = CW * 32;
-    extern __shared__ __align__(128) uint8_t smem[];
+template <int KB, int G, int GS, bool RAGGED, class EMIT>
+__device__ __forceinline__ void qk_range(Pipe& pp, Cursor& cur, const AttnParams& p, const Sched& s, int unit, int j, int left,
+                                         int n_issued, uint2* q2, float* qlin, int lane, uint64_t pol, int tl_w, EMIT&& emit)
+{
     const CacheDesc& c = p.c;
-    const int tid = threadIdx.x, warp = tid >> 5, lane = tid & 31;
     const int t4 = lane & 3;
-    const int n_stages = kCW * p.spw;
-    uint64_t* full_all = reinterpret_cast<uint64_t*>(smem + (size_t)n_stages * p.stage_bytes);
-    uint8_t* ptr = smem + (((size_t)n_stages * (p.stage_bytes + 8) + 127) & ~(size_t)127);
-    uint2* q2 = reinterpret_cast<uint2*>(ptr) + warp * (G * 32);
-    float* qlin = reinterpret_cast<float*>(ptr + kCW * G * 32 * 8) + warp * (G * kD);
-
-    __shared__ Ranges<CostQK> rg_sh;
-    const Sched s = make_sched(c);
-    if (tid < n_stages) { mbar_init(&full_all[tid], 1); mbar_fence_init(); }
-    if (tid == kThreads - 1) rg_sh.init(p.n_units, s.n_kb, s.n_kr, p.nw_eff);
-    __syncthreads();
-    pdl_trigger();
-
-    const uint64_t pol = KIVI_EVICT_FIRST ? policy_evict_first() : policy_evict_last();
-    const int gw = blockIdx.x * kCW + warp;
-    if (!sched_ok(s, c, p.max_kv_len)) { if (gw == 0 && lane == 0) c.state[6] = KIVI_STATE_ERR_CAPACITY; return; }
-    KIVI_TL(0, gw, 0);
-    const Ranges<CostQK>& rg = rg_sh;
-    if (gw >= (int)rg.W) { pdl_wait(); return; }
-    int u_lo, j_lo, u_hi, j_hi;
-    rg.lo(gw, u_lo, j_lo); rg.lo(gw + 1, u_hi, j_hi);
-    const int n_mine = (u_hi - u_lo) * s.ipu + (j_hi - j_lo);
-    Pipe pp;
-    pp.init(smem + (size_t)warp * p.spw * p.stage_bytes, full_all + warp * p.spw, p.spw, p.stage_bytes);
-    Cursor cur;
-    cur.unit = u_lo; cur.j = j_lo; cur.half = 0; cur.left = n_mine; cur.s_unit = -1; cur.s_pos = 0;
-    for (int i = 0; i < (Lat<G>::q_first ? 1 : p.spw); ++i) qk_issue_next<KB, GS, RAGGED>(pp, cur, p, s, lane, pol);
-
     constexpr int NG = Cols<G, GS>::NG;
     const int ratio = c.H / c.Hkv;
     const int h_l = t4 % G;
     const bool slow = p.mask || p.dbg_logits;
 
-    int unit = u_lo, j = j_lo, left = n_mine;
     uint2 qf[G], ql[G];
     auto fetch_q = [&](int un) {
         const int u_ = p.hchunks == 1 ? un : un / p.hchunks, hc_ = p.hchunks == 1 ? 0 : un % p.hchunks;
@@ -769,11 +760,9 @@
             ql[h] = __ldg(reinterpret_cast<const uint2*>(p.q + (int64_t)(row0 + h) * kD) + lane);
         }
     };
-    pdl_wait();
     fetch_q(unit);
-    if (Lat<G>::q_first)
-        for (int i = 1; i < p.spw; ++i) qk_issue_next<KB, GS, RAGGED>(pp, cur, p, s, lane, pol);
-    KIVI_TL(0, gw, 1);
+    for (int i = n_issued; i < p.spw; ++i) qk_issue_next<KB, GS, RAGGED>(pp, cur, p, s, lane, pol);
+    if (tl_w >= 0) KIVI_TL(0, tl_w, 1);
     #pragma unroll 1
     while (left > 0) {
         const int u = p.hchunks == 1 ? unit : unit / p.hchunks, hc = p.hchunks == 1 ? 0 : unit % p.hchunks;
@@ -920,7 +909,7 @@
             }
         }
 
-        const int w_first = rg.owner(unit, 0);
+        float M[G], S[G];
         #pragma unroll
         for (int h = 0; h < G; ++h) {
             float m = -INFINITY, sm = 0.f;
@@ -930,18 +919,63 @@
                 sm = (m == -INFINITY ? 0.f : sm * fast_exp(m - mn)) + s_blk * fast_exp(m_blk - mn);
                 m = mn;
             }
-            float M, S;
-            warp_max_sum(m, sm, M, S);
-            if (lane == 0) p.w.stats[(int64_t)(uq0 + h) * p.w.stat_cap + (gw - w_first)] = make_float2(M, S);
-        }
+            warp_max_sum(m, sm, M[h], S[h]);
+        }
+        emit(unit, uq0, M, S);
+        (void)j_first;
+        left -= n_here;
+        if (j == s.ipu) { j = 0; ++unit; }
+    }
+}
+
+template <int KB, int G, int GS, int CW, bool RAGGED>
+__global__ void __launch_bounds__(CW * 32, KIVI_MINB)
+qk_kernel(const KIVI_PARAM_QUAL AttnParams p)
+{
+    constexpr int kCW = CW, kThreads = CW * 32;
+    extern __shared__ __align__(128) uint8_t smem[];
+    const CacheDesc& c = p.c;
+    const int tid = threadIdx.x, warp = tid >> 5, lane = tid & 31;
+    const int n_stages = kCW * p.spw;
+    uint64_t* full_all = reinterpret_cast<uint64_t*>(smem + (size_t)n_stages * p.stage_bytes);
+    uint8_t* ptr = smem + (((size_t)n_stages * (p.stage_bytes + 8) + 127) & ~(size_t)127);
+    uint2* q2 = reinterpret_cast<uint2*>(ptr) + warp * (G * 32);
+    float* qlin = reinterpret_cast<float*>(ptr + kCW * G * 32 * 8) + warp * (G * kD);
+
+    __shared__ Ranges<CostQK> rg_sh;
+    const Sched s = make_sched(c);
+    if (tid < n_stages) { mbar_init(&full_all[tid], 1); mbar_fence_init(); }
+    if (tid == kThreads - 1) rg_sh.init(p.n_units, s.n_kb, s.n_kr, p.nw_eff);
+    __syncthreads();
+    pdl_trigger();
+
+    const uint64_t pol = KIVI_EVICT_FIRST ? policy_evict_first() : policy_evict_last();
+    const int gw = blockIdx.x * kCW + warp;
+    if (!sched_ok(s, c, p.max_kv_len)) { if (gw == 0 && lane == 0) c.state[6] = KIVI_STATE_ERR_CAPACITY; return; }
+    KIVI_TL(0, gw, 0);
+    const Ranges<CostQK>& rg = rg_sh;
+    if (gw >= (int)rg.W) { pdl_wait(); return; }
+    int u_lo, j_lo, u_hi, j_hi;
+    rg.lo(gw, u_lo, j_lo); rg.lo(gw + 1, u_hi, j_hi);
+    const int n_mine = (u_hi - u_lo) * s.ipu + (j_hi - j_lo);
+    Pipe pp;
+    pp.init(smem + (size_t)warp * p.spw * p.stage_bytes, full_all + warp * p.spw, p.spw, p.stage_bytes);
+    Cursor cur;
+    cur.unit = u_lo; cur.j = j_lo; cur.half = 0; cur.left = n_mine; cur.s_unit = -1; cur.s_pos = 0;
+    for (int i = 0; i < (Lat<G>::q_first ? 1 : p.spw); ++i) qk_issue_next<KB, GS, RAGGED>(pp, cur, p, s, lane, pol);
+
+    pdl_wait();
+    qk_range<KB, G, GS, RAGGED>(pp, cur, p, s, u_lo, j_lo, n_mine, Lat<G>::q_first ? 1 : p.spw, q2, qlin, lane, pol, gw,
+                                [&](int unit, int uq0, const float (&M)[G], const float (&S)[G]) {
+        const int w_first = rg.owner(unit, 0);
+        #pragma unroll
+        for (int h = 0; h < G; ++h)
+            if (lane == 0) p.w.stats[(int64_t)(uq0 + h) * p.w.stat_cap + (gw - w_first)] = make_float2(M[h], S[h]);
 #if KIVI_UNIT_FLAGS
         __syncwarp();
         if (lane == 0) asm volatile("red.release.gpu.global.add.s32 [%0], 1;" ::"l"(p.w.ready + unit) : "memory");
 #endif
-        (void)j_first;
-        left -= n_here;
-        if (j == s.ipu) { j = 0; ++unit; }
-    }
+    });
     KIVI_TL(0, gw, 2);
 #if KIVI_COMMIT_IN_QK && KIVI_EARLY_COMMIT
     {
@@ -998,7 +1032,7 @@
 #endif
 }
 
-template <int VB, int G, int GS, bool RAGGED>
+template <int VB, int G, int GS, bool RAGGED, bool WHOLE>
 __device__ __forceinline__ void sv_issue_next(Pipe& pp, Cursor& cur, const AttnParams& p, const Sched& s,
                                               int ratio, int lane, uint64_t pol, const Ranges<CostQK>& rq, int& ready_unit)
 {
@@ -1011,7 +1045,7 @@
         }
         if (cur.left <= 0) return;
     }
-    if (cur.unit != ready_unit) { wait_unit_ready(p, s, rq, cur.unit, lane); ready_unit = cur.unit; }
+    if (!WHOLE && cur.unit != ready_unit) { wait_unit_ready(p, s, rq, cur.unit, lane); ready_unit = cur.unit; }
     if (lane == 0) {
         const int u = p.hchunks == 1 ? cur.unit : cur.unit / p.hchunks, hc = p.hchunks == 1 ? 0 : cur.unit % p.hchunks;
         uint8_t* dst = pp.prod();
@@ -1057,77 +1091,47 @@
     cursor_step(cur, s.bpu, s.n_vb);
 }
 
+__device__ __forceinline__ void fold_pair(float& mx, float& sm, float2 v) {
+    const float mn = fmaxf(mx, v.x);
+    sm = (mx == -INFINITY ? 0.f : sm * fast_exp(mx - mn)) + (v.x == -INFINITY ? 0.f : v.y * fast_exp(v.x - mn));
+    mx = mn;
+}
+
 __device__ __forceinline__ float prob_f32(float x, float M, float nMl, float S, float rS) {
     const float e = fast_exp_sub(x, M, nMl);
     const float q = e * rS;
     return fmaf(fmaf(-q, S, e), rS, q);
 }
 
-template <int KB, int VB, int G, int GS, int CW, bool RAGGED>
-__global__ void __launch_bounds__(CW * 32, KIVI_MINB)
-sv_kernel(const KIVI_PARAM_QUAL AttnParams p)
-{
-    constexpr int kCW = CW, kThreads = CW * 32;
-    extern __shared__ __align__(128) uint8_t smem[];
+template <int G>
+__device__ __forceinline__ void write_out(const AttnParams& p, const Sched& s, int uq0, const float (&qs)[G][4],
+                                          const float (&rs)[G][4], int lane)
+{
+    #pragma unroll
+    for (int h = 0; h < G; ++h) {
+        __align__(8) __half o4[4];
+        #pragma unroll
+        for (int e = 0; e < 4; ++e) {
+            __half o = __float2half_rn(rs[h][e]);
+            if (s.tv > 0) o = __hadd_rn(__float2half_rn(qs[h][e]), o);
+            o4[e] = o;
+        }
+        *reinterpret_cast<uint2*>(p.out + (int64_t)(uq0 + h) * kD + lane * 4) = *reinterpret_cast<const uint2*>(o4);
+    }
+}
+
+template <int KB, int VB, int G, int GS, bool RAGGED, bool WHOLE, class PF>
+__device__ __forceinline__ void sv_range(Pipe& pp, Cursor& cur, int n_issued, const AttnParams& p, const Sched& s, int gw,
+                                         int u_lo, int j_lo, int n_mine, float* obuf, int lane, uint64_t pol,
+                                         const Ranges<CostSV>& rg, const Ranges<CostQK>& rq, const float (&Mw)[G],
+                                         const float (&Sw)[G], float* acc, int tl_w, PF&& prologue)
+{
     const CacheDesc& c = p.c;
-    const int tid = threadIdx.x, warp = tid >> 5, lane = tid & 31;
     const int t4 = lane & 3;
-    const int n_stages = kCW * p.spw;
-    uint64_t* full_all = reinterpret_cast<uint64_t*>(smem + (size_t)n_stages * p.stage_bytes);
-    uint8_t* ptr = smem + (((size_t)n_stages * (p.stage_bytes + 8) + 127) & ~(size_t)127);
-    float* obuf = reinterpret_cast<float*>(ptr) + warp * (G * kD);
+    const int ratio = c.H / c.Hkv;
     uint8_t* scratch = reinterpret_cast<uint8_t*>(obuf);
-    (void)scratch;
-
-    __shared__ Ranges<CostSV> rg_sh;
-    __shared__ Ranges<CostQK> rq_sh;
-    const Sched s = make_sched(c);
-    if (tid < n_stages) { mbar_init(&full_all[tid], 1); mbar_fence_init(); }
-    if (tid == kThreads - 1) rg_sh.init(p.n_units, s.n_vb, s.n_vr, p.nw_eff);
-    if (tid == kThreads - 33) rq_sh.init(p.n_units, s.n_kb, s.n_kr, p.nw_eff);
-    __syncthreads();
-
-    const uint64_t pol = KIVI_EVICT_FIRST ? policy_evict_first() : policy_evict_last();
-    const int gw = blockIdx.x * kCW + warp;
-    if (!sched_ok(s, c, p.max_kv_len)) return;
-    KIVI_TL(1, gw, 0);
-    const Ranges<CostSV>& rg = rg_sh;
-    const Ranges<CostQK>& rq = rq_sh;
-    if (gw >= (int)rg.W) return;
-    int u_lo, j_lo, u_hi, j_hi;
-    rg.lo(gw, u_lo, j_lo); rg.lo(gw + 1, u_hi, j_hi);
-    const int n_mine = (u_hi - u_lo) * s.bpu + (j_hi - j_lo);
-    const int ratio = c.H / c.Hkv;
-    Pipe pp;
-    pp.init(smem + (size_t)warp * p.spw * p.stage_bytes, full_all + warp * p.spw, p.spw, p.stage_bytes);
-    Cursor cur;
-    cur.unit = u_lo; cur.j = j_lo; cur.half = 0; cur.left = n_mine; cur.s_unit = -1; cur.s_pos = 0;
+    (void)scratch; (void)rg;
     int ready_unit = -1;
-    if (s.r + 1 == c.R) {
-        const int n_slices = 4 * c.B * c.Hkv, n_workers = (int)rg.W;
-        for (int sl = gw; sl < n_slices; sl += n_workers) k_flush_slice<KB>(p, s, sl >> 2, sl & 3, lane);
-    }
-#if !KIVI_COMMIT_IN_QK
-    auto commit_share = [&]() {
-        const long long nu = (long long)c.B * c.Hkv, nwk = (long long)rg.W;
-        const int u0 = (int)((gw * nu + nwk - 1) / nwk), u1 = (int)(((gw + 1) * nu + nwk - 1) / nwk);
-        for (int uu = u0; uu < u1; ++uu) commit_unit<KB, VB>(p, s, uu, lane, scratch, commit_fetch(p, s, uu, lane));
-    };
-#endif
-#if KIVI_EARLY_COMMIT && !KIVI_COMMIT_LATE && !KIVI_COMMIT_IN_QK
-#if KIVI_COMMIT_ASYNC
-    if (p.spw < 2) commit_share();
-#else
-    commit_share();
-#endif
-#endif
-#if !KIVI_UNIT_FLAGS
-    pdl_wait();
-#endif
-#if KIVI_COMMIT_IN_QK && KIVI_EARLY_COMMIT
-    if (gw == 0 && lane == 0) *p.w.ticket = 0;
-#endif
-
     constexpr int NG = Cols<G, GS>::NG;
     const int h_l = t4 % G;
     constexpr int kHalfBytes = kHalfChunks * Lay<VB>::kChunkBytes + kHalfChunks * NG * 64;
@@ -1147,11 +1151,11 @@
             if (lane < nstat) sn[h] = __ldcg(p.w.stats + (int64_t)(row0 + h) * p.w.stat_cap + lane);
         }
     };
-    fetch_stats(unit);
+    if constexpr (!WHOLE) fetch_stats(unit);
 #if KIVI_COMMIT_ASYNC && KIVI_EARLY_COMMIT && !KIVI_COMMIT_LATE && !KIVI_COMMIT_IN_QK
-    const long long cnu = (long long)c.B * c.Hkv, cnw = (long long)rg.W;
+    const long long cnu = (long long)c.B * c.Hkv, cnw = WHOLE ? 1 : (long long)rg.W;
     const int cu0 = (int)((gw * cnu + cnw - 1) / cnw), cu1 = (int)(((gw + 1) * cnu + cnw - 1) / cnw);
-    const bool commit_async = p.spw >= 2 && cu1 > cu0;
+    const bool commit_async = !WHOLE && p.spw >= 2 && cu1 > cu0;
     if (commit_async) {
         if (lane == 0) {
             uint8_t* dst = pp.prod();
@@ -1164,8 +1168,8 @@
         }
         pp.push();
     }
-    for (int i = commit_async ? 1 : 0; i < p.spw; ++i) sv_issue_next<VB, G, GS, RAGGED>(pp, cur, p, s, ratio, lane, pol, rq, ready_unit);
-    KIVI_TL(1, gw, 1);
+    for (int i = n_issued + (commit_async ? 1 : 0); i < p.spw; ++i) sv_issue_next<VB, G, GS, RAGGED, WHOLE>(pp, cur, p, s, ratio, lane, pol, rq, ready_unit);
+    if (tl_w >= 0) KIVI_TL(1, tl_w, 1);
     if (commit_async) {
         pp.wait();
         const uint8_t* st = pp.cons();
@@ -1176,17 +1180,15 @@
         if (s.L + 1 > c.R) in.vold = *reinterpret_cast<const uint2*>(st + 512 + 2 * (win_off(s.vhead, lane * 4) - s.vhead * kD));
         __syncwarp();
         pp.pop();
-        sv_issue_next<VB, G, GS, RAGGED>(pp, cur, p, s, ratio, lane, pol, rq, ready_unit);
+        sv_issue_next<VB, G, GS, RAGGED, WHOLE>(pp, cur, p, s, ratio, lane, pol, rq, ready_unit);
         commit_unit<KB, VB>(p, s, cu0, lane, scratch, in);
         for (int uu = cu0 + 1; uu < cu1; ++uu) commit_unit<KB, VB>(p, s, uu, lane, scratch, commit_fetch(p, s, uu, lane));
     }
 #else
-    for (int i = 0; i < p.spw; ++i) sv_issue_next<VB, G, GS, RAGGED>(pp, cur, p, s, ratio, lane, pol, rq, ready_unit);
-    KIVI_TL(1, gw, 1);
-#if KIVI_EARLY_COMMIT && KIVI_COMMIT_LATE && !KIVI_COMMIT_IN_QK
-    commit_share();
-#endif
-#endif
+    for (int i = n_issued; i < p.spw; ++i) sv_issue_next<VB, G, GS, RAGGED, WHOLE>(pp, cur, p, s, ratio, lane, pol, rq, ready_unit);
+    if (tl_w >= 0) KIVI_TL(1, tl_w, 1);
+#endif
+    prologue();
     int pend_unit = -1, pend_old = 0, pend_nparts = 0;
     constexpr bool kDefer = KIVI_DEFER_ARRIVE && G == 1;
     int arr_unit = -1, arr_nparts = 0;
@@ -1241,17 +1243,7 @@
                     rs[h][0] += b4[k][h].x; rs[h][1] += b4[k][h].y; rs[h][2] += b4[k][h].z; rs[h][3] += b4[k][h].w;
                 }
         }
-        #pragma unroll
-        for (int h = 0; h < G; ++h) {
-            __align__(8) __half o4[4];
-            #pragma unroll
-            for (int e = 0; e < 4; ++e) {
-                __half o = __float2half_rn(rs[h][e]);
-                if (s.tv > 0) o = __hadd_rn(__float2half_rn(qs[h][e]), o);
-                o4[e] = o;
-            }
-            *reinterpret_cast<uint2*>(p.out + (int64_t)(uq0 + h) * kD + lane * 4) = *reinterpret_cast<const uint2*>(o4);
-        }
+        write_out<G>(p, s, uq0, qs, rs, lane);
 #if !KIVI_EARLY_COMMIT
         if (hc == 0) commit_unit<KB, VB>(p, s, u, lane, scratch, cin);
 #else
@@ -1268,19 +1260,19 @@
         float M[G], S[G], rS[G], nMl[G];
         #pragma unroll
         for (int h = 0; h < G; ++h) {
+            if constexpr (WHOLE) { M[h] = Mw[h]; S[h] = Sw[h]; }
+            else {
             float mx = sn[h].x, sm = sn[h].y;
             const float2* st = p.w.stats + (int64_t)(uq0 + h) * p.w.stat_cap;
             for (int i = lane + 32; i < nstat; i += 32) {
-                const float2 v = __ldcg(st + i);
-                const float mn = fmaxf(mx, v.x);
-                sm = (mx == -INFINITY ? 0.f : sm * fast_exp(mx - mn)) + (v.x == -INFINITY ? 0.f : v.y * fast_exp(v.x - mn));
-                mx = mn;
+                fold_pair(mx, sm, __ldcg(st + i));
             }
             warp_max_sum(mx, sm, M[h], S[h]);
+            }
             nMl[h] = -M[h] * kLog2e;
             rS[h] = __frcp_rn(S[h]);
         }
-        if (left > n_here) fetch_stats(unit + 1);
+        if (!WHOLE && left > n_here) fetch_stats(unit + 1);
 
         float run[Slots<G, GS>::k];
         float orr[G][4];
@@ -1369,7 +1361,7 @@
                     }, acc, zc, lane);
                     __syncwarp();
                     pp.pop();
-                    sv_issue_next<VB, G, GS, RAGGED>(pp, cur, p, s, ratio, lane, pol, rq, ready_unit);
+                    sv_issue_next<VB, G, GS, RAGGED, WHOLE>(pp, cur, p, s, ratio, lane, pol, rq, ready_unit);
                 }
                 float zsel[NG];
                 gather_z<G, GS>(zc, lane, zsel);
@@ -1438,7 +1430,7 @@
                 }
                 __syncwarp();
                 pp.pop();
-                sv_issue_next<VB, G, GS, RAGGED>(pp, cur, p, s, ratio, lane, pol, rq, ready_unit);
+                sv_issue_next<VB, G, GS, RAGGED, WHOLE>(pp, cur, p, s, ratio, lane, pol, rq, ready_unit);
                 #pragma unroll
                 for (int mt = 0; mt < 8; ++mt)
                     #pragma unroll
@@ -1471,34 +1463,230 @@
             if (kDefer && arr_unit >= 0) { do_arrive(arr_unit, arr_nparts); arr_unit = -1; }
         }
 
-        const int w_first = rg.owner(unit, 0), w_last = rg.owner(unit, s.bpu - 1);
-        const int nparts = w_last - w_first + 1;
-        float* recp = p.w.part + ((int64_t)unit * p.w.part_cap + (gw - w_first)) * rec;
-        {
-            float* rq = recp + (h_l * 2 + 0) * kD;
-            walk_slots<G, GS>(run, lane, [&](int o, float v) { rq[o] = v * kProbScaleInv; });
+        if constexpr (WHOLE) {
+            walk_slots<G, GS>(run, lane, [&](int o, float v) { obuf[h_l * kD + o] = v * kProbScaleInv; });
+            __syncwarp();
             #pragma unroll
-            for (int h = 0; h < G; ++h)
-                *reinterpret_cast<float4*>(recp + (h * 2 + 1) * kD + lane * 4) = make_float4(orr[h][0], orr[h][1], orr[h][2], orr[h][3]);
-        }
-        if (pend_unit >= 0 && __shfl_sync(0xffffffffu, pend_old, 0) == pend_nparts - 1) finish_unit(pend_unit, pend_nparts, pend_cin);
-        pend_unit = -1;
-#if !KIVI_EARLY_COMMIT
-        pend_cin = commit_fetch(p, s, u, lane);
-#endif
-        if (nparts > 1) {
-            if (kDefer && left > n_here) { arr_unit = unit; arr_nparts = nparts; }
-            else do_arrive(unit, nparts);
+            for (int h = 0; h < G; ++h) {
+                const float4 a = *reinterpret_cast<const float4*>(obuf + h * kD + lane * 4);
+                float4* qa = reinterpret_cast<float4*>(acc + (h * 2 + 0) * kD + lane * 4);
+                float4* ra = reinterpret_cast<float4*>(acc + (h * 2 + 1) * kD + lane * 4);
+                float4 q = *qa, r = *ra;
+                q.x += a.x; q.y += a.y; q.z += a.z; q.w += a.w;
+                r.x += orr[h][0]; r.y += orr[h][1]; r.z += orr[h][2]; r.w += orr[h][3];
+                *qa = q; *ra = r;
+            }
+            __syncwarp();
+            (void)uq0;
         } else {
-            __syncwarp();
-            finish_unit(unit, 1, pend_cin);
+            const int w_first = rg.owner(unit, 0), w_last = rg.owner(unit, s.bpu - 1);
+            const int nparts = w_last - w_first + 1;
+            float* recp = p.w.part + ((int64_t)unit * p.w.part_cap + (gw - w_first)) * rec;
+            {
+                float* rq = recp + (h_l * 2 + 0) * kD;
+                walk_slots<G, GS>(run, lane, [&](int o, float v) { rq[o] = v * kProbScaleInv; });
+                #pragma unroll
+                for (int h = 0; h < G; ++h)
+                    *reinterpret_cast<float4*>(recp + (h * 2 + 1) * kD + lane * 4) = make_float4(orr[h][0], orr[h][1], orr[h][2], orr[h][3]);
+            }
+            if (pend_unit >= 0 && __shfl_sync(0xffffffffu, pend_old, 0) == pend_nparts - 1) finish_unit(pend_unit, pend_nparts, pend_cin);
+            pend_unit = -1;
+    #if !KIVI_EARLY_COMMIT
+            pend_cin = commit_fetch(p, s, u, lane);
+    #endif
+            if (nparts > 1) {
+                if (kDefer && left > n_here) { arr_unit = unit; arr_nparts = nparts; }
+                else do_arrive(unit, nparts);
+            } else {
+                __syncwarp();
+                finish_unit(unit, 1, pend_cin);
+            }
         }
         left -= n_here;
         if (j == s.bpu) { j = 0; ++unit; }
     }
-    KIVI_TL(1, gw, 2);
+    if (tl_w >= 0) KIVI_TL(1, tl_w, 2);
     if (pend_unit >= 0 && __shfl_sync(0xffffffffu, pend_old, 0) == pend_nparts - 1) finish_unit(pend_unit, pend_nparts, pend_cin);
-    KIVI_TL(1, gw, 3);
+    if (tl_w >= 0) KIVI_TL(1, tl_w, 3);
+}
+
+template <int KB, int VB, int G, int GS, int CW, bool RAGGED>
+__global__ void __launch_bounds__(CW * 32, KIVI_MINB)
+sv_kernel(const KIVI_PARAM_QUAL AttnParams p)
+{
+    constexpr int kCW = CW, kThreads = CW * 32;
+    extern __shared__ __align__(128) uint8_t smem[];
+    const CacheDesc& c = p.c;
+    const int tid = threadIdx.x, warp = tid >> 5, lane = tid & 31;
+    const int n_stages = kCW * p.spw;
+    uint64_t* full_all = reinterpret_cast<uint64_t*>(smem + (size_t)n_stages * p.stage_bytes);
+    uint8_t* ptr = smem + (((size_t)n_stages * (p.stage_bytes + 8) + 127) & ~(size_t)127);
+    float* obuf = reinterpret_cast<float*>(ptr) + warp * (G * kD);
+    uint8_t* scratch = reinterpret_cast<uint8_t*>(obuf);
+    (void)scratch;
+
+    __shared__ Ranges<CostSV> rg_sh;
+    __shared__ Ranges<CostQK> rq_sh;
+    const Sched s = make_sched(c);
+    if (tid < n_stages) { mbar_init(&full_all[tid], 1); mbar_fence_init(); }
+    if (tid == kThreads - 1) rg_sh.init(p.n_units, s.n_vb, s.n_vr, p.nw_eff);
+    if (tid == kThreads - 33) rq_sh.init(p.n_units, s.n_kb, s.n_kr, p.nw_eff);
+    __syncthreads();
+
+    const uint64_t pol = KIVI_EVICT_FIRST ? policy_evict_first() : policy_evict_last();
+    const int gw = blockIdx.x * kCW + warp;
+    if (!sched_ok(s, c, p.max_kv_len)) return;
+    KIVI_TL(1, gw, 0);
+    const Ranges<CostSV>& rg = rg_sh;
+    const Ranges<CostQK>& rq = rq_sh;
+    if (gw >= (int)rg.W) return;
+    int u_lo, j_lo, u_hi, j_hi;
+    rg.lo(gw, u_lo, j_lo); rg.lo(gw + 1, u_hi, j_hi);
+    const int n_mine = (u_hi - u_lo) * s.bpu + (j_hi - j_lo);
+    Pipe pp;
+    pp.init(smem + (size_t)warp * p.spw * p.stage_bytes, full_all + warp * p.spw, p.spw, p.stage_bytes);
+    if (s.r + 1 == c.R) {
+        const int n_slices = 4 * c.B * c.Hkv, n_workers = (int)rg.W;
+        for (int sl = gw; sl < n_slices; sl += n_workers) k_flush_slices<KB, 1>(p, s, sl >> 2, sl & 3, lane);
+    }
+#if !KIVI_COMMIT_IN_QK
+    auto commit_share = [&]() {
+        const long long nu = (long long)c.B * c.Hkv, nwk = (long long)rg.W;
+        const int u0 = (int)((gw * nu + nwk - 1) / nwk), u1 = (int)(((gw + 1) * nu + nwk - 1) / nwk);
+        for (int uu = u0; uu < u1; ++uu) commit_unit<KB, VB>(p, s, uu, lane, scratch, commit_fetch(p, s, uu, lane));
+    };
+#endif
+#if KIVI_EARLY_COMMIT && !KIVI_COMMIT_LATE && !KIVI_COMMIT_IN_QK
+#if KIVI_COMMIT_ASYNC
+    if (p.spw < 2) commit_share();
+#else
+    commit_share();
+#endif
+#endif
+#if !KIVI_UNIT_FLAGS
+    pdl_wait();
+#endif
+#if KIVI_COMMIT_IN_QK && KIVI_EARLY_COMMIT
+    if (gw == 0 && lane == 0) *p.w.ticket = 0;
+#endif
+
+    Cursor cur;
+    cur.unit = u_lo; cur.j = j_lo; cur.half = 0; cur.left = n_mine; cur.s_unit = -1; cur.s_pos = 0;
+    const float none[G] = {};
+    sv_range<KB, VB, G, GS, RAGGED, false>(pp, cur, 0, p, s, gw, u_lo, j_lo, n_mine, obuf, lane, pol, rg, rq, none, none,
+                                           nullptr, gw, [&]() {
+#if KIVI_EARLY_COMMIT && KIVI_COMMIT_LATE && !KIVI_COMMIT_IN_QK
+        commit_share();
+#endif
+    });
+}
+
+template <class C>
+__device__ __noinline__ int2 unit_piece(const Ranges<C>& rg, int unit, int k)
+{
+    const int w0 = rg.owner(unit, 0);
+    if (k < 0) return make_int2(w0, rg.owner(unit, rg.per_unit - 1));
+    int ua, ja, ub, jb;
+    rg.lo(w0 + k, ua, ja); rg.lo(w0 + k + 1, ub, jb);
+    return make_int2(ua == unit ? ja : 0, ub == unit ? jb : rg.per_unit);
+}
+
+template <int KB, int VB, int G, int GS, int CW>
+__global__ void __launch_bounds__(CW * 32, 1)
+unit_kernel(const KIVI_PARAM_QUAL AttnParams p)
+{
+    static_assert(G == 1, "the whole-unit kernel serves one query head per unit");
+    extern __shared__ __align__(128) uint8_t smem[];
+    const CacheDesc& c = p.c;
+    const int tid = threadIdx.x, warp = tid >> 5, lane = tid & 31;
+    const int n_stages = CW * p.spw;
+    uint64_t* full_all = reinterpret_cast<uint64_t*>(smem + (size_t)n_stages * p.stage_bytes);
+    uint8_t* ptr = smem + (((size_t)n_stages * (p.stage_bytes + 8) + 127) & ~(size_t)127);
+    uint2* q2 = reinterpret_cast<uint2*>(ptr) + warp * (G * 32);
+    float* qlin = reinterpret_cast<float*>(ptr + CW * G * 32 * 8) + warp * (G * kD);
+    float* obuf = reinterpret_cast<float*>(ptr + CW * G * (32 * 8 + kD * 4)) + warp * (G * kD);
+    float* acc = reinterpret_cast<float*>(ptr + CW * G * (32 * 8 + 2 * kD * 4)) + warp * (G * 2 * kD);
+
+    __shared__ Ranges<CostQK> rq_sh;
+    __shared__ Ranges<CostSV> rv_sh;
+    const Sched s = make_sched(c);
+    if (tid < n_stages) { mbar_init(&full_all[tid], 1); mbar_fence_init(); }
+    if (tid == CW * 32 - 1) rq_sh.init(p.n_units, s.n_kb, s.n_kr, p.nw_eff);
+    if (tid == CW * 32 - 33) rv_sh.init(p.n_units, s.n_vb, s.n_vr, p.nw_eff);
+    __syncthreads();
+
+    const uint64_t pol = KIVI_EVICT_FIRST ? policy_evict_first() : policy_evict_last();
+    const int gw = blockIdx.x * CW + warp, W = gridDim.x * CW;
+    if (!sched_ok(s, c, p.max_kv_len)) { if (gw == 0 && lane == 0) c.state[6] = KIVI_STATE_ERR_CAPACITY; return; }
+    KIVI_TL(0, gw, 0);
+    if (gw >= p.n_units) { pdl_wait(); return; }
+    Pipe pp;
+    pp.init(smem + (size_t)warp * p.spw * p.stage_bytes, full_all + warp * p.spw, p.spw, p.stage_bytes);
+    const Ranges<CostQK>& rq = rq_sh;
+    const Ranges<CostSV>& rv = rv_sh;
+    const bool flush = s.r + 1 == c.R;
+    #pragma unroll 1
+    for (int unit = gw; unit < p.n_units; unit += W) {
+        Cursor cur;
+        cur.unit = unit; cur.j = 0; cur.half = 0; cur.left = s.ipu; cur.s_unit = -1; cur.s_pos = 0;
+        int n_issued = unit == gw && Lat<G>::q_first ? 1 : p.spw;
+        for (int i = 0; i < n_issued; ++i) qk_issue_next<KB, GS, false>(pp, cur, p, s, lane, pol);
+        if (unit == gw) pdl_wait();
+        float mx[G], sm[G];
+        #pragma unroll
+        for (int h = 0; h < G; ++h) { mx[h] = -INFINITY; sm[h] = 0.f; }
+        const int2 wq = unit_piece(rq, unit, -1);
+        #pragma unroll 1
+        for (int k = 0; k <= wq.y - wq.x; ++k) {
+            const int2 jr = unit_piece(rq, unit, k);
+            const int j0 = jr.x, j1 = jr.y;
+            qk_range<KB, G, GS, false>(pp, cur, p, s, unit, j0, j1 - j0, n_issued, q2, qlin, lane, pol,
+                                       unit == gw && k == 0 ? gw : -1, [&](int, int, const float (&Mu)[G], const float (&Su)[G]) {
+                #pragma unroll
+                for (int h = 0; h < G; ++h) {
+                    if (k < 32) { if (lane == k) { mx[h] = Mu[h]; sm[h] = Su[h]; } }
+                    else if (lane == (k & 31)) fold_pair(mx[h], sm[h], make_float2(Mu[h], Su[h]));
+                }
+            });
+            n_issued = p.spw;
+        }
+        float M[G], S[G];
+        #pragma unroll
+        for (int h = 0; h < G; ++h) warp_max_sum(mx[h], sm[h], M[h], S[h]);
+        if (unit == gw) KIVI_TL(0, gw, 2);
+        asm volatile("fence.proxy.async.global;" ::: "memory");
+        __syncwarp();
+        Cursor vcur;
+        vcur.unit = unit; vcur.j = 0; vcur.half = 0; vcur.left = s.bpu; vcur.s_unit = -1; vcur.s_pos = 0;
+        #pragma unroll
+        for (int h = 0; h < 2 * G; ++h) *reinterpret_cast<float4*>(acc + h * kD + lane * 4) = make_float4(0.f, 0.f, 0.f, 0.f);
+        const int2 wv = unit_piece(rv, unit, -1);
+        #pragma unroll 1
+        for (int k = 0; k <= wv.y - wv.x; ++k) {
+            const int2 jr = unit_piece(rv, unit, k);
+            const int j0 = jr.x, j1 = jr.y;
+            const bool first = k == 0;
+            sv_range<KB, VB, G, GS, false, true>(pp, vcur, first ? 0 : p.spw, p, s, gw, unit, j0, j1 - j0, obuf, lane, pol, rv, rq,
+                                                 M, S, acc, -1, [&]() {
+                if (!first || unit % p.hchunks != 0) return;
+                const int u = unit / p.hchunks;
+                if (flush) k_flush_slices<KB, 4>(p, s, u, 0, lane);
+                commit_unit<KB, VB>(p, s, u, lane, reinterpret_cast<uint8_t*>(obuf), commit_fetch(p, s, u, lane));
+            });
+        }
+        float qs[G][4], rs[G][4];
+        constexpr int kBatch = G == 1 ? 4 : 2;
+        const float pad = (wv.y - wv.x + 1) % kBatch != 0 ? 0.f : -0.f;
+        #pragma unroll
+        for (int h = 0; h < G; ++h) {
+            const float4 q = *reinterpret_cast<const float4*>(acc + (h * 2 + 0) * kD + lane * 4);
+            const float4 r = *reinterpret_cast<const float4*>(acc + (h * 2 + 1) * kD + lane * 4);
+            qs[h][0] = q.x + pad; qs[h][1] = q.y + pad; qs[h][2] = q.z + pad; qs[h][3] = q.w + pad;
+            rs[h][0] = r.x + pad; rs[h][1] = r.y + pad; rs[h][2] = r.z + pad; rs[h][3] = r.w + pad;
+        }
+        write_out<G>(p, s, (unit / p.hchunks) * (c.H / c.Hkv) + (unit % p.hchunks) * G, qs, rs, lane);
+    }
+    KIVI_TL(0, gw, 3);
 }
 
 constexpr int kMaxCtasPerSm = KIVI_MINB;
@@ -1534,6 +1722,47 @@
     return off;
 }
 
+constexpr int kUnitCW = 8;
+constexpr double kUnitFill = 0.9;
+enum { kPathAuto = 0, kPathTwoLaunch = 1, kPathUnit = 2 };
+int& attention_path_force();
+__host__ inline int attention_path(int n_units, int num_sms, int G, bool ragged, int force)
+{
+    const bool eligible = !ragged && G == 1 && n_units > 0 && num_sms > 0;
+    if (!eligible) return kPathTwoLaunch;
+    if (force == kPathTwoLaunch || force == kPathUnit) return force;
+    const long long W = (long long)num_sms * kUnitCW;
+    return n_units <= W && (double)n_units >= kUnitFill * (double)W ? kPathUnit : kPathTwoLaunch;
+}
+
+template <int KB, int VB, int G, int GS>
+static int launch_unit(AttnParams& p, const DeviceInfo& di, bool overlap_prologue, cudaStream_t st)
+{
+    const Tuning& tn = tuning();
+    const int max_smem = di.max_smem_optin - 1024;
+    const int half_k = kHalfChunks * Lay<KB>::kChunkBytes + lay_meta_bytes(GS);
+    const int half_v = kHalfChunks * Lay<VB>::kChunkBytes + lay_meta_bytes(GS) + G * kPartTokens * 2;
+    const int stage = max(max(half_k, half_v), kResBytes + G * 64);
+    p.stage_bytes = (stage + 127) / 128 * 128;
+    const int fixed = 512 + kUnitCW * G * (32 * 8 + 4 * kD * 4);
+    p.spw = min(8, (max_smem - fixed) / (kUnitCW * p.stage_bytes));
+    if (tn.stages_per_warp >= 1 && tn.stages_per_warp <= p.spw) p.spw = tn.stages_per_warp;
+    if (p.spw < 1) return KIVI_ERR_CAPACITY;
+    const size_t smem = (size_t)kUnitCW * p.spw * p.stage_bytes + fixed;
+    auto ku = unit_kernel<KB, VB, G, GS, kUnitCW>;
+    static std::atomic<unsigned long long> optin{0};
+    int rc = ensure_dynamic_smem(ku, max_smem, di.ordinal, optin); if (rc) return rc;
+    cudaLaunchAttribute attr[1];
+    attr[0].id = cudaLaunchAttributeProgrammaticStreamSerialization;
+    attr[0].val.programmaticStreamSerializationAllowed = !tn.no_pdl && overlap_prologue ? 1 : 0;
+    cudaLaunchConfig_t cfg = {};
+    cfg.gridDim = dim3(di.num_sms); cfg.blockDim = dim3(kUnitCW * 32); cfg.dynamicSmemBytes = smem; cfg.stream = st;
+    cfg.attrs = attr; cfg.numAttrs = 1;
+    const cudaError_t e = cudaLaunchKernelEx(&cfg, ku, p);
+    if (e != cudaSuccess) return (int)e;
+    return post_launch();
+}
+
 template <int KB, int VB, int G, int GS, bool RAGGED>
 static int launch_attention(AttnParams& p, bool overlap_prologue, cudaStream_t st)
 {
@@ -1571,6 +1800,10 @@
     const int grid = di.num_sms * ctas;
     const long long want = (long long)p.n_units * max(1, p.w.part_cap - 2);
     p.nw_eff = (int)min((long long)grid * kCW, want);
+    if constexpr (!RAGGED && G == 1) {
+        if (attention_path(p.n_units, di.num_sms, G, RAGGED, attention_path_force()) == kPathUnit)
+            return launch_unit<KB, VB, G, GS>(p, di, overlap_prologue, st);
+    }
     const bool pdl = !tn.no_pdl;
     cudaLaunchAttribute attr_qk[1], attr_sv[1];
     attr_qk[0].id = attr_sv[0].id = cudaLaunchAttributeProgrammaticStreamSerialization;
diff --git a/kivi_b200/csrc/kivi_decode.cu b/kivi_b200/csrc/kivi_decode.cu
--- a/kivi_b200/csrc/kivi_decode.cu
+++ b/kivi_b200/csrc/kivi_decode.cu
@@ -141,6 +141,23 @@
     return run(rg);
 }
 
+namespace kivi {
+int& attention_path_force() { static int mode = kPathAuto; return mode; }
+}
+
+extern "C" int kivi_debug_attention_path(int n_units, int num_sms, int G, int ragged)
+{
+    return attention_path(n_units, num_sms, G, ragged != 0, attention_path_force());
+}
+
+extern "C" int kivi_debug_force_attention_path(int mode)
+{
+    if (mode != kPathAuto && mode != kPathTwoLaunch && mode != kPathUnit) return KIVI_ERR_SHAPE;
+    const int prev = attention_path_force();
+    attention_path_force() = mode;
+    return prev;
+}
+
 #if KIVI_TIMELINE
 #include <vector>
 namespace kivi {
```

Measured after the change: 2933 (median of 6 runs). +3.6%, better.
